# hangxu0304/DeepReduce

Hardware: NVIDIA H100
Metric: ResNet-50 images/sec (whole job, device-timed, max over ranks) (higher is better)
Workload: dtype bf16

## Files before the change

### deepreduce_b200/models/fused_bn.py

```python
from __future__ import annotations

import os

import torch
import torch.nn as nn
import torch.nn.functional as F


def enabled() -> bool:
    return os.environ.get("DR_FUSED_BN", "1") != "0"


def _eligible_x(x: torch.Tensor) -> bool:
    return (x.is_cuda and x.dtype == torch.bfloat16 and x.dim() == 4 and x.stride(1) == 1
            and x.is_contiguous(memory_format=torch.channels_last) and x.size(1) % 8 == 0 and x.size(1) <= 8192
            and x.numel() < 2 ** 31 - 1 and x.numel() // x.size(1) > 1)


def _eligible_bn(bn: nn.BatchNorm2d) -> bool:
    return (bn.training and bn.track_running_stats and bn.running_mean is not None and bn.momentum is not None
            and bn.affine)


def eligible(x: torch.Tensor, bn: nn.BatchNorm2d) -> bool:
    return enabled() and _eligible_x(x) and _eligible_bn(bn)


def _stats(x, bn):
    from .. import ops
    bn.num_batches_tracked.add_(1)
    return ops.cuda_module().bn_stats(x, bn.running_mean, bn.running_var, float(bn.momentum), float(bn.eps))


def _grad(go):
    return go.contiguous(memory_format=torch.channels_last)


def _fork(ctx, o, fork):
    if not fork:
        return o
    ctx.set_materialize_grads(False)
    return o, o.detach()


def _grads(grads):
    gs = [_grad(g) for g in grads if g is not None]
    return (gs + [None, None])[:2]


class _BNReLU(torch.autograd.Function):
    @staticmethod
    def forward(ctx, x, weight, bias, mean, invstd):
        from .. import ops
        y, mask = ops.cuda_module().bn_apply(0, x, [mean, invstd, weight, bias])
        ctx.save_for_backward(x, weight, mean, invstd, mask)
        return y

    @staticmethod
    def backward(ctx, gy):
        from .. import ops
        x, weight, mean, invstd, mask = ctx.saved_tensors
        dx, dw, db = ops.cuda_module().bn_backward(0, _grad(gy), mask, x, [mean, invstd, weight])
        return dx, dw, db, None, None


class _BNAddReLU(torch.autograd.Function):

    @staticmethod
    def forward(ctx, x, weight, bias, mean, invstd, z, wz, bz, mz, iz, fork):
        from .. import ops
        mod = ops.cuda_module()
        if wz is None:
            o, mask = mod.bn_apply(1, x, [mean, invstd, weight, bias], z)
            ctx.save_for_backward(x, weight, mean, invstd, mask)
        else:
            o, mask = mod.bn_apply(2, x, [mean, invstd, weight, bias], z, [mz, iz, wz, bz])
            ctx.save_for_backward(x, weight, mean, invstd, mask, z, wz, mz, iz)
        ctx.has_bn_z = wz is not None
        return _fork(ctx, o, fork)

    @staticmethod
    def backward(ctx, *grads):
        from .. import ops
        mod = ops.cuda_module()
        go, go2 = _grads(grads)
        if go is None:
            return (None,) * 11
        saved = ctx.saved_tensors
        x, weight, mean, invstd, mask = saved[:5]
        if not ctx.has_bn_z:
            dx, dw, db, g = mod.bn_backward(1, go, mask, x, [mean, invstd, weight], go2=go2)
            return dx, dw, db, None, None, g, None, None, None, None, None
        z, wz, mz, iz = saved[5:]
        dx, dw, db, dz, dwz, dbz = mod.bn_backward(2, go, mask, x, [mean, invstd, weight], z, [mz, iz, wz], go2=go2)
        return dx, dw, db, None, None, dz, dwz, dbz, None, None, None


class _BNReLUMaxPool(torch.autograd.Function):

    @staticmethod
    def forward(ctx, x, weight, bias, mean, invstd, fork):
        from .. import ops
        out, codes = ops.cuda_module().bn_apply_pool(x, [mean, invstd, weight, bias])
        ctx.save_for_backward(x, weight, mean, invstd, codes)
        return _fork(ctx, out, fork)

    @staticmethod
    def backward(ctx, *grads):
        from .. import ops
        go, go2 = _grads(grads)
        if go is None:
            return (None,) * 6
        x, weight, mean, invstd, codes = ctx.saved_tensors
        dx, dw, db = ops.cuda_module().bn_backward(3, go, codes, x, [mean, invstd, weight], go2=go2)
        return dx, dw, db, None, None, None


def _stem_pool(pool: nn.Module) -> bool:
    if type(pool) is not nn.MaxPool2d:
        return False
    pair = lambda v: tuple(v) if isinstance(v, (tuple, list)) else (v, v)
    return (pair(pool.kernel_size) == (3, 3) and pair(pool.stride) == (2, 2) and pair(pool.padding) == (1, 1)
            and pair(pool.dilation) == (1, 1) and not pool.ceil_mode and not pool.return_indices)


def _pair(o, fork):
    return (o, o) if fork else o


def bn_relu_maxpool(x: torch.Tensor, bn: nn.BatchNorm2d, pool: nn.MaxPool2d, fork: bool = False):
    if not (eligible(x, bn) and _stem_pool(pool)):
        return _pair(pool(F.relu(bn(x), inplace=True)), fork)
    mean, invstd = _stats(x, bn)
    return _BNReLUMaxPool.apply(x, bn.weight, bn.bias, mean, invstd, fork)


def bn_relu(x: torch.Tensor, bn: nn.BatchNorm2d) -> torch.Tensor:
    if not eligible(x, bn):
        return F.relu(bn(x), inplace=True)
    mean, invstd = _stats(x, bn)
    return _BNReLU.apply(x, bn.weight, bn.bias, mean, invstd)


def bn_add_relu(x: torch.Tensor, bn: nn.BatchNorm2d, idt: torch.Tensor, fork: bool = False):
    if not (eligible(x, bn) and idt.dtype == x.dtype and idt.shape == x.shape and idt.stride() == x.stride()):
        return _pair(F.relu(bn(x) + idt, inplace=True), fork)
    mean, invstd = _stats(x, bn)
    return _BNAddReLU.apply(x, bn.weight, bn.bias, mean, invstd, idt, None, None, None, None, fork)


def bn_bn_add_relu(x: torch.Tensor, bn: nn.BatchNorm2d, xd: torch.Tensor, bnd: nn.BatchNorm2d, fork: bool = False):
    if not (eligible(x, bn) and eligible(xd, bnd) and xd.shape == x.shape and xd.stride() == x.stride()):
        return _pair(F.relu(bn(x) + bnd(xd), inplace=True), fork)
    md, id_ = _stats(xd, bnd)
    mean, invstd = _stats(x, bn)
    return _BNAddReLU.apply(x, bn.weight, bn.bias, mean, invstd, xd, bnd.weight, bnd.bias, md, id_, fork)
```

### deepreduce_b200/models/resnet.py

```python
from __future__ import annotations

import torch.nn as nn
import torch.nn.functional as F

from .fused_bn import bn_add_relu, bn_bn_add_relu, bn_relu, bn_relu_maxpool


class _BasicCifar(nn.Module):
    def __init__(self, inp, out, stride):
        super().__init__()
        self.conv1 = nn.Conv2d(inp, out, 3, stride, 1, bias=False)
        self.bn1 = nn.BatchNorm2d(out)
        self.conv2 = nn.Conv2d(out, out, 3, 1, 1, bias=False)
        self.bn2 = nn.BatchNorm2d(out)
        self.pad = None
        if stride != 1 or inp != out:
            self.pad = (out - inp, stride)

    def forward(self, x):
        y = F.relu(self.bn1(self.conv1(x)))
        y = self.bn2(self.conv2(y))
        if self.pad is not None:
            extra, s = self.pad
            x = F.pad(x[:, :, ::s, ::s], (0, 0, 0, 0, extra // 2, extra - extra // 2))
        return F.relu(x + y)


class ResNetCifar(nn.Module):
    def __init__(self, n: int = 3, num_classes: int = 10):
        super().__init__()
        self.conv1 = nn.Conv2d(3, 16, 3, 1, 1, bias=False)
        self.bn1 = nn.BatchNorm2d(16)
        layers, inp = [], 16
        for out, stride in ((16, 1), (32, 2), (64, 2)):
            for i in range(n):
                layers.append(_BasicCifar(inp, out, stride if i == 0 else 1))
                inp = out
        self.layers = nn.Sequential(*layers)
        self.fc = nn.Linear(64, num_classes)

    def forward(self, x):
        x = F.relu(self.bn1(self.conv1(x)))
        x = self.layers(x)
        x = F.adaptive_avg_pool2d(x, 1).flatten(1)
        return self.fc(x)


def resnet20(num_classes: int = 10) -> ResNetCifar:
    return ResNetCifar(3, num_classes)


class _Bottleneck(nn.Module):
    expansion = 4

    def __init__(self, inp, width, stride, downsample):
        super().__init__()
        out = width * self.expansion
        self.conv1 = nn.Conv2d(inp, width, 1, bias=False)
        self.bn1 = nn.BatchNorm2d(width)
        self.conv2 = nn.Conv2d(width, width, 3, stride, 1, bias=False)
        self.bn2 = nn.BatchNorm2d(width)
        self.conv3 = nn.Conv2d(width, out, 1, bias=False)
        self.bn3 = nn.BatchNorm2d(out)
        self.downsample = None
        if downsample:
            self.downsample = nn.Sequential(nn.Conv2d(inp, out, 1, stride, bias=False), nn.BatchNorm2d(out))

    def forward(self, x, skip=None, fork=False):
        skip = x if skip is None else skip
        xd = None if self.downsample is None else self.downsample[0](skip)
        y = bn_relu(self.conv1(x), self.bn1)
        y = bn_relu(self.conv2(y), self.bn2)
        y = self.conv3(y)
        if xd is None:
            return bn_add_relu(y, self.bn3, skip, fork=fork)
        o = bn_bn_add_relu(y, self.bn3, xd, self.downsample[1])
        return (o, None) if fork else o


class ResNet(nn.Module):
    def __init__(self, blocks=(3, 4, 6, 3), num_classes: int = 1000):
        super().__init__()
        self.conv1 = nn.Conv2d(3, 64, 7, 2, 3, bias=False)
        self.bn1 = nn.BatchNorm2d(64)
        self.maxpool = nn.MaxPool2d(3, 2, 1)
        stages, inp = [], 64
        for i, (n, width) in enumerate(zip(blocks, (64, 128, 256, 512))):
            for j in range(n):
                stride = 2 if (j == 0 and i > 0) else 1
                stages.append(_Bottleneck(inp, width, stride, downsample=(j == 0)))
                inp = width * 4
        self.layers = nn.Sequential(*stages)
        self.fc = nn.Linear(inp, num_classes)
        for m in self.modules():
            if isinstance(m, nn.Conv2d):
                nn.init.kaiming_normal_(m.weight, mode="fan_out", nonlinearity="relu")

    def forward(self, x):
        x, skip = bn_relu_maxpool(self.conv1(x), self.bn1, self.maxpool), None
        for blk in self.layers:
            x, skip = blk(x, skip, fork=True)
        x = F.adaptive_avg_pool2d(x, 1).flatten(1)
        return self.fc(x)


def resnet50(num_classes: int = 1000) -> ResNet:
    return ResNet((3, 4, 6, 3), num_classes)
```

### deepreduce_b200/ops/build.py

```python
from __future__ import annotations

import hashlib
import os
import shutil
import subprocess
import sysconfig
from concurrent.futures import ThreadPoolExecutor

HERE = os.path.dirname(os.path.abspath(__file__))
CSRC = os.path.join(HERE, "csrc")
OBJ = os.path.join(HERE, "build")

CUDA_SOURCES = ["engine.cu", "ops.cu", "p2p.cu", "bn.cu", "p2.cu", "repack.cu"]
NVCC_FLAGS = ["-gencode", "arch=compute_90a,code=sm_90a", "-lineinfo", "-O3", "-std=c++17",
              "--expt-relaxed-constexpr", "--expt-extended-lambda", "-Xcompiler", "-fPIC", "-Xptxas", "-v"]


def _run(cmd, log=None):
    r = subprocess.run(cmd, stdout=subprocess.PIPE, stderr=subprocess.STDOUT, text=True)
    if log is not None:
        with open(log, "w") as f:
            f.write(" ".join(cmd) + "\n" + r.stdout)
    if r.returncode != 0:
        raise RuntimeError("command failed:\n" + " ".join(cmd) + "\n" + r.stdout[-6000:])
    return r.stdout


def _stale(target, sources, extra=""):
    stamp = target + ".stamp"
    h = hashlib.sha256(extra.encode())
    for s in sources:
        with open(s, "rb") as f:
            h.update(f.read())
    digest = h.hexdigest()
    if os.path.exists(target) and os.path.exists(stamp) and open(stamp).read() == digest:
        return False, digest, stamp
    return True, digest, stamp


def _headers():
    return [os.path.join(CSRC, f) for f in os.listdir(CSRC) if f.endswith((".h", ".cuh"))]


def build_cpu(verbose=True):
    import pybind11
    src = os.path.join(CSRC, "cpu", "native_cpu.cpp")
    out = os.path.join(HERE, "_dr_cpu.so")
    stale, digest, stamp = _stale(out, [src])
    if not stale:
        return out
    os.makedirs(OBJ, exist_ok=True)
    cmd = ["g++", "-O3", "-std=c++17", "-shared", "-fPIC", "-fvisibility=hidden",
           "-I", pybind11.get_include(), "-I", sysconfig.get_paths()["include"], src, "-o", out]
    _run(cmd, os.path.join(OBJ, "cpu.log"))
    open(stamp, "w").write(digest)
    if verbose:
        print(f"[build] {out}")
    return out


def build_cuda(verbose=True):
    import torch
    from torch.utils import cpp_extension as ce
    nvcc = shutil.which("nvcc") or "/usr/local/cuda/bin/nvcc"
    out = os.path.join(HERE, "_dr_cuda.so")
    srcs = [os.path.join(CSRC, s) for s in CUDA_SOURCES] + [os.path.join(CSRC, "binding.cpp")]
    stale, digest, stamp = _stale(out, srcs + _headers(), extra=torch.__version__ + " ".join(NVCC_FLAGS))
    if not stale:
        return out
    os.makedirs(OBJ, exist_ok=True)
    abi = int(torch._C._GLIBCXX_USE_CXX11_ABI)

    def cu(src):
        o = os.path.join(OBJ, os.path.basename(src) + ".o")
        _run([nvcc] + NVCC_FLAGS + ["-I", CSRC, "-c", src, "-o", o], os.path.join(OBJ, os.path.basename(src) + ".log"))
        return o

    def cpp(src):
        o = os.path.join(OBJ, "binding.o")
        inc = []
        for p in ce.include_paths("cuda"):
            inc += ["-isystem", p]
        cmd = ["g++", "-O2", "-std=c++17", "-fPIC", "-c", src, "-o", o, "-I", CSRC,
               "-I", sysconfig.get_paths()["include"], f"-D_GLIBCXX_USE_CXX11_ABI={abi}",
               "-DTORCH_EXTENSION_NAME=_dr_cuda", "-DTORCH_API_INCLUDE_EXTENSION_H", "-w"] + inc
        _run(cmd, os.path.join(OBJ, "binding.log"))
        return o

    with ThreadPoolExecutor(max_workers=4) as ex:
        futs = [ex.submit(cu, s) for s in srcs[:-1]] + [ex.submit(cpp, srcs[-1])]
        objs = [f.result() for f in futs]
    libdirs = ce.library_paths("cuda")
    link = ["g++", "-shared", "-o", out] + objs
    for d in libdirs:
        link += ["-L", d, f"-Wl,-rpath,{d}"]
    link += ["-lc10", "-lc10_cuda", "-ltorch_cpu", "-ltorch_cuda", "-ltorch", "-ltorch_python", "-lcudart"]
    _run(link, os.path.join(OBJ, "link.log"))
    open(stamp, "w").write(digest)
    if verbose:
        print(f"[build] {out}")
    return out


def build_all(verbose=True):
    return build_cpu(verbose), build_cuda(verbose)


if __name__ == "__main__":
    build_all()
    for f in sorted(os.listdir(OBJ)):
        if f.endswith(".cu.log"):
            txt = open(os.path.join(OBJ, f)).read()
            for line in txt.splitlines():
                if "registers" in line or "Compiling entry" in line or "spill" in line:
                    print(line)
```

### deepreduce_b200/ops/csrc/binding.cpp

```cpp
#include <ATen/cuda/CUDAContext.h>
#include <c10/cuda/CUDAGuard.h>
#include <c10/cuda/CUDAStream.h>
#include <torch/extension.h>

#include <algorithm>
#include <condition_variable>
#include <deque>
#include <mutex>
#include <thread>

#include "ops.h"

namespace py = pybind11;
using dr::EngineParams;

#define CHECK_CUDA_T(x) TORCH_CHECK((x).is_cuda() && (x).is_contiguous(), #x " must be a contiguous CUDA tensor")

static cudaStream_t cur_stream() { return at::cuda::getCurrentCUDAStream().stream(); }

static void check_last(const char* what) {
  cudaError_t e = cudaGetLastError();
  TORCH_CHECK(e == cudaSuccess, what, ": ", cudaGetErrorString(e));
}

static torch::Tensor bloom_insert(torch::Tensor idx, int64_t k, int64_t m_bits, int64_t seed) {
  CHECK_CUDA_T(idx);
  TORCH_CHECK(idx.scalar_type() == torch::kInt64, "idx must be int64");
  c10::cuda::CUDAGuard g(idx.device());
  const int64_t n_words = (m_bits + 31) / 32;
  auto words = torch::zeros({n_words}, idx.options().dtype(torch::kInt32));
  dr::launch_bloom_insert(idx.data_ptr<int64_t>(), idx.numel(), (uint32_t*)words.data_ptr<int32_t>(), (uint32_t)k,
                          (uint32_t)m_bits, (uint32_t)seed, cur_stream());
  check_last("bloom_insert");
  return words;
}

static torch::Tensor bloom_select(torch::Tensor words, int64_t d, int64_t limit, int64_t k, int64_t m_bits, int64_t seed) {
  CHECK_CUDA_T(words);
  c10::cuda::CUDAGuard g(words.device());
  const int64_t n_tiles = (d + dr::kTile - 1) / dr::kTile;
  auto opts32 = words.options().dtype(torch::kInt32);
  auto counts = torch::empty({n_tiles}, opts32);
  auto excl = torch::empty({n_tiles + 1}, opts32);
  const uint32_t* f = (const uint32_t*)words.data_ptr<int32_t>();
  dr::launch_bloom_count(f, (uint32_t)d, (uint32_t)k, (uint32_t)m_bits, (uint32_t)seed,
                         (uint32_t*)counts.data_ptr<int32_t>(), (uint32_t*)excl.data_ptr<int32_t>(), cur_stream());
  const int64_t total = excl[n_tiles].item<int32_t>();
  const int64_t n_out = (limit < 0) ? total : std::min<int64_t>(limit, total);
  auto out = torch::empty({n_out}, words.options().dtype(torch::kInt64));
  if (n_out > 0)
    dr::launch_bloom_emit(f, (uint32_t)d, (uint32_t)k, (uint32_t)m_bits, (uint32_t)seed,
                          (const uint32_t*)excl.data_ptr<int32_t>(), out.data_ptr<int64_t>(), (uint32_t)n_out, cur_stream());
  check_last("bloom_select");
  return out;
}

static std::vector<torch::Tensor> qsgd_encode(torch::Tensor vals, int64_t q, int64_t bucket, int64_t seed) {
  CHECK_CUDA_T(vals);
  c10::cuda::CUDAGuard g(vals.device());
  auto v = vals.to(torch::kFloat32).contiguous();
  const int64_t K = v.numel();
  const bool i16 = q >= 128;
  auto lvl = torch::empty({K}, v.options().dtype(i16 ? torch::kInt16 : torch::kInt8));
  auto norms = torch::empty({(K + bucket - 1) / bucket}, v.options());
  dr::launch_qsgd_encode(v.data_ptr<float>(), K, (int)bucket, (int)q, (uint32_t)seed, lvl.data_ptr(), i16,
                         norms.data_ptr<float>(), cur_stream());
  check_last("qsgd_encode");
  return {lvl, norms};
}

static torch::Tensor qsgd_decode(torch::Tensor lvl, torch::Tensor norms, int64_t q, int64_t bucket) {
  CHECK_CUDA_T(lvl); CHECK_CUDA_T(norms);
  c10::cuda::CUDAGuard g(lvl.device());
  const bool i16 = lvl.scalar_type() == torch::kInt16;
  auto out = torch::empty({lvl.numel()}, norms.options());
  dr::launch_qsgd_decode(lvl.data_ptr(), i16, norms.data_ptr<float>(), lvl.numel(), (int)bucket, (int)q,
                         out.data_ptr<float>(), cur_stream());
  check_last("qsgd_decode");
  return out;
}

static torch::Tensor pack_bits(torch::Tensor vals, int64_t bits) {
  CHECK_CUDA_T(vals);
  TORCH_CHECK(1 <= bits && bits <= 63, "pack_bits: bits must be in [1, 63], got ", bits);
  c10::cuda::CUDAGuard g(vals.device());
  auto v = vals.to(torch::kInt64).contiguous();
  const int64_t n = v.numel();
  const int64_t n_bytes = (n * bits + 7) / 8, n_words = (n * bits + 31) / 32;
  auto out = torch::empty({n_words}, v.options().dtype(torch::kInt32));
  dr::launch_pack_bits(v.data_ptr<int64_t>(), n, (int)bits, (uint32_t*)out.data_ptr<int32_t>(), n_words, cur_stream());
  check_last("pack_bits");
  return out.view(torch::kUInt8).slice(0, 0, n_bytes);
}

static torch::Tensor unpack_bits(torch::Tensor buf, int64_t n, int64_t bits) {
  CHECK_CUDA_T(buf);
  TORCH_CHECK(1 <= bits && bits <= 63, "unpack_bits: bits must be in [1, 63], got ", bits);
  c10::cuda::CUDAGuard g(buf.device());
  const int64_t n_words = (n * bits + 31) / 32;
  auto padded = torch::zeros({n_words * 4}, buf.options().dtype(torch::kUInt8));
  padded.slice(0, 0, buf.numel()).copy_(buf);
  auto out = torch::empty({n}, buf.options().dtype(torch::kInt64));
  dr::launch_unpack_bits((const uint32_t*)padded.data_ptr<uint8_t>(), n_words, n, (int)bits, out.data_ptr<int64_t>(),
                         cur_stream());
  check_last("unpack_bits");
  return out;
}

static torch::Tensor polyfit_fit(torch::Tensor y, torch::Tensor seg_off, torch::Tensor seg_len, int64_t degree, int64_t max_seg) {
  CHECK_CUDA_T(y); CHECK_CUDA_T(seg_off); CHECK_CUDA_T(seg_len);
  c10::cuda::CUDAGuard g(y.device());
  auto coeffs = torch::zeros({max_seg * (degree + 1)}, y.options());
  dr::launch_polyfit_fit(y.data_ptr<float>(), seg_off.data_ptr<int>(), seg_len.data_ptr<int>(), (int)seg_len.numel(),
                         (int)degree, coeffs.data_ptr<float>(), cur_stream());
  check_last("polyfit_fit");
  return coeffs;
}

static torch::Tensor polyfit_eval(torch::Tensor coeffs, torch::Tensor seg_off, torch::Tensor seg_len, int64_t degree, int64_t total) {
  CHECK_CUDA_T(coeffs);
  c10::cuda::CUDAGuard g(coeffs.device());
  auto out = torch::empty({total}, coeffs.options());
  dr::launch_polyfit_eval(coeffs.data_ptr<float>(), seg_off.data_ptr<int>(), seg_len.data_ptr<int>(),
                          (int)seg_len.numel(), (int)degree, total, out.data_ptr<float>(), cur_stream());
  check_last("polyfit_eval");
  return out;
}

static torch::Tensor conflict_sets_pick(torch::Tensor set_off, torch::Tensor members, torch::Tensor last, int64_t n_pos, int64_t K,
                                        int64_t pseed) {
  CHECK_CUDA_T(set_off); CHECK_CUDA_T(members); CHECK_CUDA_T(last);
  c10::cuda::CUDAGuard g(set_off.device());
  auto out = torch::zeros({(n_pos + 31) / 32}, set_off.options().dtype(torch::kInt32));
  cudaError_t e = dr::launch_conflict_sets_pick((const uint32_t*)set_off.data_ptr<int32_t>(), (const uint32_t*)members.data_ptr<int32_t>(),
                                                (uint32_t*)last.data_ptr<int32_t>(), (uint32_t)(set_off.numel() - 1), (uint32_t)n_pos,
                                                (uint32_t)K, (uint32_t)pseed, (uint32_t*)out.data_ptr<int32_t>(), cur_stream());
  TORCH_CHECK(e == cudaSuccess, "conflict_sets_pick: ", cudaGetErrorString(e));
  return out;
}

static torch::Tensor dexp_fit(torch::Tensor y) {
  CHECK_CUDA_T(y);
  c10::cuda::CUDAGuard g(y.device());
  auto v = y.to(torch::kFloat32).contiguous();
  auto out = torch::zeros({4}, v.options().dtype(torch::kFloat64));
  dr::launch_dexp_fit(v.data_ptr<float>(), v.numel(), out.data_ptr<double>(), cur_stream());
  check_last("dexp_fit");
  return out;
}

static torch::Tensor delta_bp128_encode(torch::Tensor idx) {
  CHECK_CUDA_T(idx);
  c10::cuda::CUDAGuard g(idx.device());
  const int64_t n = idx.numel();
  const int64_t nb = (n + 127) / 128;
  auto widths = torch::zeros({nb}, idx.options().dtype(torch::kInt32));
  dr::launch_bp128_widths(idx.data_ptr<int64_t>(), n, (uint32_t*)widths.data_ptr<int32_t>(), cur_stream());
  auto sizes = widths.to(torch::kInt64) * 4 + 1;
  auto incl = sizes.cumsum(0);
  auto off = (incl - sizes).contiguous();
  const int64_t total = nb ? incl[nb - 1].item<int64_t>() : 0;
  auto out = torch::zeros({total}, idx.options().dtype(torch::kInt32));
  dr::launch_bp128_pack(idx.data_ptr<int64_t>(), n, (const uint32_t*)widths.data_ptr<int32_t>(), off.data_ptr<int64_t>(),
                        (uint32_t*)out.data_ptr<int32_t>(), cur_stream());
  check_last("delta_bp128_encode");
  return out;
}

static torch::Tensor delta_bp128_decode(torch::Tensor payload, int64_t n) {
  CHECK_CUDA_T(payload);
  c10::cuda::CUDAGuard g(payload.device());
  const int64_t nb = (n + 127) / 128;
  auto off = torch::empty({nb + 1}, payload.options().dtype(torch::kInt64));
  auto deltas = torch::empty({n}, payload.options().dtype(torch::kInt64));
  dr::launch_bp128_unpack((const uint32_t*)payload.data_ptr<int32_t>(), n, off.data_ptr<int64_t>(),
                          deltas.data_ptr<int64_t>(), cur_stream());
  check_last("delta_bp128_decode");
  return deltas.cumsum(0);
}

static torch::Tensor rle_runs(torch::Tensor idx, int64_t d) {
  CHECK_CUDA_T(idx);
  c10::cuda::CUDAGuard g(idx.device());
  const int64_t n = idx.numel();
  auto o64 = idx.options().dtype(torch::kInt64);
  if (n == 0) return torch::full({1}, d, o64);
  const int64_t nb = (n + 1023) / 1024;
  auto counts = torch::empty({nb}, idx.options().dtype(torch::kInt32));
  auto excl = torch::empty({nb + 1}, idx.options().dtype(torch::kInt32));
  dr::launch_rle_count(idx.data_ptr<int64_t>(), n, (uint32_t*)counts.data_ptr<int32_t>(), (uint32_t*)excl.data_ptr<int32_t>(),
                       cur_stream());
  const int64_t n_runs = excl[nb].item<int32_t>();
  auto start_pos = torch::empty({n_runs}, o64), end_pos = torch::empty({n_runs}, o64);
  auto runs = torch::zeros({2 * n_runs + 1}, o64);
  dr::launch_rle_runs(idx.data_ptr<int64_t>(), n, (const uint32_t*)excl.data_ptr<int32_t>(), start_pos.data_ptr<int64_t>(),
                      end_pos.data_ptr<int64_t>(), n_runs, d, runs.data_ptr<int64_t>(), cur_stream());
  check_last("rle_runs");
  const int64_t last = idx[n - 1].item<int64_t>();
  return (d - 1 - last > 0) ? runs : runs.slice(0, 0, 2 * n_runs);
}

static torch::Tensor rle_indices(torch::Tensor runs) {
  CHECK_CUDA_T(runs);
  c10::cuda::CUDAGuard g(runs.device());
  const int64_t n_pairs = runs.numel() / 2;
  auto o64 = runs.options().dtype(torch::kInt64);
  if (n_pairs == 0) return torch::empty({0}, o64);
  auto pairs = runs.slice(0, 0, 2 * n_pairs).to(torch::kInt64).view({n_pairs, 2});
  auto z = pairs.select(1, 0), o = pairs.select(1, 1);
  auto csum = (z + o).cumsum(0);
  auto run_start = (csum - o).contiguous();
  auto ones_incl = o.cumsum(0);
  auto ones_excl = (ones_incl - o).contiguous();
  const int64_t total = ones_incl[n_pairs - 1].item<int64_t>();
  auto out = torch::empty({total}, o64);
  dr::launch_rle_expand(ones_excl.data_ptr<int64_t>(), run_start.data_ptr<int64_t>(), n_pairs, total, out.data_ptr<int64_t>(),
                        cur_stream());
  check_last("rle_indices");
  return out;
}

static torch::Tensor u8_to_nhwc_norm(torch::Tensor in, std::vector<double> mean, std::vector<double> stdv) {
  CHECK_CUDA_T(in);
  TORCH_CHECK(in.scalar_type() == torch::kUInt8 && in.size(-1) == 3, "expect uint8 [...,3] NHWC");
  c10::cuda::CUDAGuard g(in.device());
  in = in.contiguous();
  if (reinterpret_cast<uintptr_t>(in.data_ptr()) % 4 != 0) in = in.clone(at::MemoryFormat::Contiguous);
  auto out = torch::empty(in.sizes(), in.options().dtype(torch::kBFloat16));
  float m[3] = {(float)mean[0], (float)mean[1], (float)mean[2]};
  float s[3] = {(float)(1.0 / stdv[0]), (float)(1.0 / stdv[1]), (float)(1.0 / stdv[2])};
  dr::launch_u8_to_nhwc_norm(in.data_ptr<uint8_t>(), out.data_ptr(), in.numel() / 3, m, s, cur_stream());
  check_last("u8_to_nhwc_norm");
  return out;
}

struct Repack {
  torch::Tensor table;
  int64_t n_seg = 0, n_vec = 0, ddp_numel = 0, eng_numel = 0;
  int elem_bytes = 0;
  c10::ScalarType dtype;

  Repack(torch::Tensor segs, int64_t ddp_numel_, int64_t eng_numel_, torch::Tensor like)
      : ddp_numel(ddp_numel_), eng_numel(eng_numel_), dtype(like.scalar_type()) {
    TORCH_CHECK(dtype == torch::kFloat32 || dtype == torch::kBFloat16, "Repack: fp32 or bf16 buckets, got ", dtype);
    TORCH_CHECK(like.is_cuda(), "Repack: the buckets must be CUDA tensors");
    const torch::Device device = like.device();
    TORCH_CHECK(!segs.is_cuda() && segs.scalar_type() == torch::kInt64 && segs.dim() == 2 && segs.size(1) == 3,
                "Repack: segments must be a host int64 tensor [n, 3] of {ddp_off, eng_off, numel}");
    elem_bytes = dtype == torch::kFloat32 ? 4 : 2;
    const int64_t V = 16 / elem_bytes;
    segs = segs.contiguous();
    n_seg = segs.size(0);
    TORCH_CHECK(n_seg < (1 << 30), "Repack: too many segments");
    auto host = torch::empty({n_seg + 1, 4}, torch::kInt64);
    const int64_t* s = segs.data_ptr<int64_t>();
    int64_t* h = host.data_ptr<int64_t>();
    std::vector<std::pair<int64_t, int64_t>> ddp_ranges, eng_ranges;
    for (int64_t i = 0; i < n_seg; ++i) {
      const int64_t d = s[3 * i], e = s[3 * i + 1], n = s[3 * i + 2];
      TORCH_CHECK(n > 0, "Repack: segment ", i, " is empty");
      TORCH_CHECK(d >= 0 && d + n <= ddp_numel, "Repack: segment ", i, " [", d, ", ", d + n,
                  ") lies outside the DDP buffer of ", ddp_numel, " elements");
      TORCH_CHECK(e >= 0 && e % V == 0, "Repack: segment ", i, " starts at engine element ", e,
                  ", not on a 16-byte vector");
      TORCH_CHECK((e + n + V - 1) / V * V <= eng_numel, "Repack: segment ", i, " [", e, ", ", e + n,
                  ") lies outside the engine buffer of ", eng_numel, " elements");
      h[4 * i] = d; h[4 * i + 1] = e; h[4 * i + 2] = n; h[4 * i + 3] = n_vec;
      n_vec += (n + V - 1) / V;
      ddp_ranges.emplace_back(d, d + n);
      eng_ranges.emplace_back(e, e + n);
    }
    h[4 * n_seg] = 0; h[4 * n_seg + 1] = 0; h[4 * n_seg + 2] = 0; h[4 * n_seg + 3] = n_vec;
    for (auto* r : {&ddp_ranges, &eng_ranges}) {
      std::sort(r->begin(), r->end());
      for (size_t i = 1; i < r->size(); ++i)
        TORCH_CHECK((*r)[i].first >= (*r)[i - 1].second, "Repack: segments overlap at element ", (*r)[i].first);
    }
    table = host.to(device);
  }

  void check_buffers(const torch::Tensor& ddp, const torch::Tensor& eng) const {
    for (const torch::Tensor* t : {&ddp, &eng}) {
      TORCH_CHECK(t->is_cuda() && t->is_contiguous() && t->dim() == 1, "Repack: buffers are contiguous 1-D CUDA tensors");
      TORCH_CHECK(t->scalar_type() == dtype, "Repack: the table was built for ", dtype, " buffers, got ", t->scalar_type());
      TORCH_CHECK(t->device() == table.device(), "Repack: buffer on ", t->device(), ", table on ", table.device());
    }
    TORCH_CHECK(ddp.numel() >= ddp_numel, "Repack: the DDP buffer has ", ddp.numel(), " elements, the table needs ", ddp_numel);
    TORCH_CHECK(eng.numel() >= eng_numel, "Repack: the engine buffer has ", eng.numel(), " elements, the table needs ", eng_numel);
    TORCH_CHECK(reinterpret_cast<uintptr_t>(eng.data_ptr()) % 16 == 0, "Repack: the engine buffer must be 16-byte aligned");
  }

  void pack(torch::Tensor ddp, torch::Tensor eng) const {
    check_buffers(ddp, eng);
    c10::cuda::CUDAGuard g(eng.device());
    cudaError_t e = dr::launch_bucket_repack(true, elem_bytes, ddp.data_ptr(), eng.data_ptr(), table.data_ptr<int64_t>(),
                                             (int)n_seg, n_vec, cur_stream());
    TORCH_CHECK(e == cudaSuccess, "bucket_pack: ", cudaGetErrorString(e));
  }

  void unpack(torch::Tensor eng, torch::Tensor ddp) const {
    check_buffers(ddp, eng);
    c10::cuda::CUDAGuard g(eng.device());
    cudaError_t e = dr::launch_bucket_repack(false, elem_bytes, eng.data_ptr(), ddp.data_ptr(), table.data_ptr<int64_t>(),
                                             (int)n_seg, n_vec, cur_stream());
    TORCH_CHECK(e == cudaSuccess, "bucket_unpack: ", cudaGetErrorString(e));
  }
};

namespace at::native {
struct Var;
template <typename scalar_t, typename VarTransform>
void batch_norm_stats_channels_last_cuda_template(const at::Tensor& out_mean, const at::Tensor& out_invstd,
                                                   const at::Tensor& input, double epsilon);
}

static void check_bn_input(const torch::Tensor& x) {
  TORCH_CHECK(x.is_cuda() && x.scalar_type() == torch::kBFloat16 && x.dim() == 4 && x.stride(1) == 1 &&
                  x.is_contiguous(at::MemoryFormat::ChannelsLast),
              "bn: x must be a channels_last bf16 CUDA tensor");
  TORCH_CHECK(x.size(1) % 8 == 0 && x.size(1) <= 8192, "bn: channels must be a multiple of 8, at most 8192");
  TORCH_CHECK(x.numel() < std::numeric_limits<int32_t>::max(), "bn: tensor too large for 32-bit indexing");
}

static void check_chan(const torch::Tensor& t, int64_t C, const char* what) {
  TORCH_CHECK(t.is_cuda() && t.scalar_type() == torch::kFloat32 && t.is_contiguous() && t.numel() == C, "bn: ", what,
              " must be a contiguous float32 CUDA tensor of C elements");
}

static std::vector<torch::Tensor> bn_stats(torch::Tensor x, torch::Tensor running_mean, torch::Tensor running_var,
                                           double momentum, double eps, bool torch_kernel) {
  check_bn_input(x);
  const int64_t C = x.size(1);
  check_chan(running_mean, C, "running_mean");
  check_chan(running_var, C, "running_var");
  const int64_t N = x.numel() / C;
  TORCH_CHECK(N > 1, "bn: expected more than 1 value per channel when training");
  c10::cuda::CUDAGuard g(x.device());
  auto opts = x.options().dtype(torch::kFloat32);
  auto mean = torch::empty({C}, opts), invstd = torch::empty({C}, opts);
  const float bessel = static_cast<float>(static_cast<double>(N) / static_cast<double>(N - 1));
  int block_y = 0, grid_y = 0;
  dr::bn_row_tree(N, (int)C, &block_y, &grid_y);
  cudaError_t e;
  if (!torch_kernel && (int64_t)block_y * grid_y <= N) {
    auto staging = grid_y > 1 ? torch::empty({(2 * C + 1) * grid_y}, opts) : torch::Tensor();
    const dr::BnStats s{x.data_ptr(), mean.data_ptr<float>(), invstd.data_ptr<float>(), running_mean.data_ptr<float>(),
                        running_var.data_ptr<float>(), grid_y > 1 ? staging.data_ptr<float>() : nullptr,
                        (float)momentum, bessel, (float)eps};
    e = dr::launch_bn_stats(s, N, (int)C, cur_stream());
  } else {
    at::native::batch_norm_stats_channels_last_cuda_template<c10::BFloat16, at::native::Var>(mean, invstd, x, eps);
    e = dr::launch_bn_update_stats(mean.data_ptr<float>(), invstd.data_ptr<float>(), running_mean.data_ptr<float>(),
                                   running_var.data_ptr<float>(), (int)C, (float)momentum, bessel, (float)eps,
                                   cur_stream());
  }
  TORCH_CHECK(e == cudaSuccess, "bn_stats: ", cudaGetErrorString(e));
  return {mean, invstd};
}

static dr::BnParams bn_params(const std::vector<torch::Tensor>& p, int64_t C) {
  TORCH_CHECK(p.size() == 4, "bn: expected (mean, invstd, weight, bias)");
  const char* names[4] = {"mean", "invstd", "weight", "bias"};
  for (int i = 0; i < 4; ++i) check_chan(p[i], C, names[i]);
  return {p[0].data_ptr<float>(), p[1].data_ptr<float>(), p[2].data_ptr<float>(), p[3].data_ptr<float>()};
}

static void check_like_x(const torch::Tensor& t, const torch::Tensor& x, const char* what) {
  TORCH_CHECK(t.sizes() == x.sizes() && t.strides() == x.strides() && t.scalar_type() == torch::kBFloat16 &&
                  t.device() == x.device(),
              "bn: ", what, " must match x in shape, layout, dtype and device");
}

static std::vector<torch::Tensor> bn_apply(int64_t mode, torch::Tensor x, std::vector<torch::Tensor> p,
                                           c10::optional<torch::Tensor> z, std::vector<torch::Tensor> pz) {
  check_bn_input(x);
  const int64_t C = x.size(1);
  const dr::BnParams px = bn_params(p, C);
  dr::BnParams pzz{};
  const void* zp = nullptr;
  if (mode != 0) {
    TORCH_CHECK(z.has_value(), "bn: mode ", mode, " needs z");
    check_like_x(*z, x, "z");
    zp = z->data_ptr();
    if (mode == 2) pzz = bn_params(pz, C);
  }
  c10::cuda::CUDAGuard g(x.device());
  const int64_t rows = x.numel() / C;
  auto out = torch::empty_like(x);
  auto mask = torch::empty({rows, C / 8}, x.options().dtype(torch::kUInt8));
  cudaError_t e = dr::launch_bn_apply((int)mode, x.data_ptr(), px, zp, pzz, out.data_ptr(), mask.data_ptr(), rows,
                                      (int)C, cur_stream());
  TORCH_CHECK(e == cudaSuccess, "bn_apply: ", cudaGetErrorString(e));
  return {out, mask};
}

static std::vector<torch::Tensor> bn_apply_pool(torch::Tensor x, std::vector<torch::Tensor> p, int64_t kernel_size,
                                                int64_t stride, int64_t padding, int64_t dilation, bool ceil_mode) {
  TORCH_CHECK(kernel_size == 3 && stride == 2 && padding == 1 && dilation == 1 && !ceil_mode,
              "bn_apply_pool: only kernel 3, stride 2, padding 1, dilation 1, floor mode");
  check_bn_input(x);
  const int64_t N = x.size(0), C = x.size(1), H = x.size(2), W = x.size(3);
  const dr::BnParams px = bn_params(p, C);
  c10::cuda::CUDAGuard g(x.device());
  const dr::PoolGeom pg{(int)H, (int)W, (int)((H - 1) / 2 + 1), (int)((W - 1) / 2 + 1)};
  auto out = torch::empty({N, C, pg.Ho, pg.Wo}, x.options().memory_format(at::MemoryFormat::ChannelsLast));
  auto codes = torch::empty({N * pg.Ho * pg.Wo, C}, x.options().dtype(torch::kUInt8));
  cudaError_t e = dr::launch_bn_apply_pool(x.data_ptr(), px, out.data_ptr(), codes.data_ptr(), (int)N, pg, (int)C,
                                           cur_stream());
  TORCH_CHECK(e == cudaSuccess, "bn_apply_pool: ", cudaGetErrorString(e));
  return {out, codes};
}

static dr::BnParams bn_bwd_params(const std::vector<torch::Tensor>& p, int64_t C) {
  TORCH_CHECK(p.size() == 3, "bn_backward: expected (mean, invstd, weight)");
  const char* names[3] = {"mean", "invstd", "weight"};
  for (int i = 0; i < 3; ++i) check_chan(p[i], C, names[i]);
  return {p[0].data_ptr<float>(), p[1].data_ptr<float>(), p[2].data_ptr<float>(), nullptr};
}

static std::vector<torch::Tensor> bn_backward(int64_t mode, torch::Tensor go, torch::Tensor mask, torch::Tensor x,
                                              std::vector<torch::Tensor> p, c10::optional<torch::Tensor> z,
                                              std::vector<torch::Tensor> pz, c10::optional<torch::Tensor> go2) {
  TORCH_CHECK(mode >= 0 && mode <= 3, "bn_backward: mode must be 0, 1, 2 or 3");
  TORCH_CHECK(!go2.has_value() || mode != 0, "bn_backward: mode 0 takes no go2");
  check_bn_input(x);
  const int64_t C = x.size(1), rows = x.numel() / C;
  dr::PoolGeom pg{(int)x.size(2), (int)x.size(3), (int)((x.size(2) - 1) / 2 + 1), (int)((x.size(3) - 1) / 2 + 1)};
  const std::vector<int64_t> go_shape =
      mode == 3 ? std::vector<int64_t>{x.size(0), C, pg.Ho, pg.Wo} : x.sizes().vec();
  for (const torch::Tensor* t : {&go, go2.has_value() ? &*go2 : &go})
    TORCH_CHECK(t->sizes() == go_shape && t->scalar_type() == torch::kBFloat16 && t->device() == x.device() &&
                    t->is_contiguous(at::MemoryFormat::ChannelsLast),
                "bn_backward: go and go2 must be channels_last bf16 tensors on x's device, of x's shape (mode 3: the "
                "pooled shape)");
  const int64_t mask_numel = mode == 3 ? go.numel() : rows * (C / 8);
  TORCH_CHECK(mask.is_cuda() && mask.scalar_type() == torch::kUInt8 && mask.is_contiguous() &&
                  mask.numel() == mask_numel && mask.device() == x.device(),
              "bn_backward: mask must be bn_apply's mask (mode 3: bn_apply_pool's codes) for x");
  c10::cuda::CUDAGuard guard(x.device());
  int block_y = 0, grid_y = 0;
  dr::bn_row_tree(rows, (int)C, &block_y, &grid_y);
  TORCH_CHECK((int64_t)block_y * grid_y <= rows, "bn_backward: reduction tree wider than the rows");
  const int n_sums = mode == 2 ? 3 : 2;
  auto f32 = x.options().dtype(torch::kFloat32);
  auto sums = torch::empty({n_sums, C}, f32);
  auto staging = grid_y > 1 ? torch::empty({n_sums, grid_y, C}, f32) : torch::Tensor();
  auto dx = torch::empty_like(x), dw = torch::empty({C}, f32), db = torch::empty({C}, f32);
  dr::BnBwd b{};
  b.go = go.data_ptr(); b.go2 = go2.has_value() ? go2->data_ptr() : nullptr; b.mask = mask.data_ptr<uint8_t>(); b.x = x.data_ptr();
  b.px = bn_bwd_params(p, C);
  b.dx = dx.data_ptr(); b.sums = sums.data_ptr<float>(); b.staging = grid_y > 1 ? staging.data_ptr<float>() : nullptr;
  b.dw = dw.data_ptr<float>(); b.db = db.data_ptr<float>();
  b.pool = pg;
  std::vector<torch::Tensor> res{dx, dw, db};
  torch::Tensor g;
  if (mode == 1 || mode == 3) {
    g = torch::empty_like(x);
    b.g = g.data_ptr();
    if (mode == 1) res.push_back(g);
  } else if (mode == 2) {
    TORCH_CHECK(z.has_value(), "bn_backward: mode 2 needs z");
    check_like_x(*z, x, "z");
    b.z = z->data_ptr();
    b.pz = bn_bwd_params(pz, C);
    auto dz = torch::empty_like(x), dwz = torch::empty({C}, f32), dbz = torch::empty({C}, f32);
    b.dz = dz.data_ptr(); b.dwz = dwz.data_ptr<float>(); b.dbz = dbz.data_ptr<float>();
    res.insert(res.end(), {dz, dwz, dbz});
  }
  cudaError_t e = dr::launch_bn_backward((int)mode, b, rows, (int)C, cur_stream());
  TORCH_CHECK(e == cudaSuccess, "bn_backward: ", cudaGetErrorString(e));
  return res;
}

struct Engine {
  EngineParams P{};
  int grid = 0;
  int grid_cap = 0;
  int blocks_per_sm = 2;
  int dyn_smem = 64 * 1024;
  int device = 0;
  const dr::P2Entry* p2_entries = nullptr;
  uint32_t n_p2 = 0, p2_max_pos_cap = 0;
  uint32_t* p2_scratch = nullptr;

  Engine(int64_t tensors, int64_t tiles, int64_t n_tensors, int64_t n_tiles, int64_t slot_words,
         int64_t payload_words, int64_t grad, int64_t resid, int64_t hist, int64_t hist_total, int64_t sel,
         int64_t tile_count, int64_t barrier, int64_t status, std::vector<int64_t> arenas, int rank, int world) {
    TORCH_CHECK(world <= dr::kMaxWorld && (int)arenas.size() == world, "bad world/arenas");
    P.tensors = reinterpret_cast<const dr::TensorDesc*>(tensors);
    P.tiles = reinterpret_cast<const dr::TileInfo*>(tiles);
    P.n_tensors = (uint32_t)n_tensors; P.n_tiles = (uint32_t)n_tiles;
    P.slot_words = (uint32_t)slot_words; P.payload_words = (uint32_t)payload_words;
    P.grad = reinterpret_cast<float*>(grad); P.resid = reinterpret_cast<float*>(resid);
    P.hist = reinterpret_cast<uint32_t*>(hist); P.hist_total = reinterpret_cast<uint32_t*>(hist_total);
    P.sel = reinterpret_cast<dr::SelState*>(sel);
    P.tile_count = reinterpret_cast<uint32_t*>(tile_count);
    P.barrier = reinterpret_cast<uint32_t*>(barrier); P.status = reinterpret_cast<uint32_t*>(status);
    for (int i = 0; i < world; ++i) P.arena[i] = reinterpret_cast<uint32_t*>(arenas[i]);
    P.rank = rank; P.world = world;
    P.beta = 1.f; P.gamma = 1.f; P.scale = 1.f / world; P.seed = dr::kDefaultSeed; P.policy = 0; P.use_history = 1;
    P.spin_limit = 20u * 1000u * 1000u;
    P.filter_smem_words = (uint32_t)(dyn_smem / 4);
    P.use_tma = 1; P.hist_shift = 23;
    P.shard = 0; P.s2_words = 0; P.s2_cap = 0; P.has_rle = 0; P.has_shared = 0; P.has_bf16_values = 0; P.mc_arena = nullptr;
    P.peer_timeout_ms = 120000u; P.fault = 0; P.debug_times = nullptr; P.cost_prefix = nullptr; P.deterministic = 0; P.cuts = nullptr; P.cuts_grid = 0;
    cudaGetDevice(&device);
  }

  void configure(double beta, double gamma, double scale, int64_t seed, int policy, int use_history, int64_t spin_limit,
                 int bps, int64_t filter_smem_bytes, int use_tma, int hist_shift) {
    P.beta = (float)beta; P.gamma = (float)gamma; P.scale = (float)scale; P.seed = (uint32_t)seed;
    P.policy = policy; P.use_history = use_history; P.spin_limit = (uint32_t)spin_limit;
    blocks_per_sm = bps; grid = 0;
    dyn_smem = (int)filter_smem_bytes; P.filter_smem_words = (uint32_t)(dyn_smem / 4);
    P.use_tma = use_tma; P.hist_shift = (uint32_t)hist_shift;
  }

  void set_poly(int64_t tensors, int64_t n_poly, int64_t tasks, int64_t n_tasks, int64_t bins, int64_t bucket_val,
                int64_t bucket_pos, int64_t expand_buf, int64_t poly_total) {
    P.poly_tensors = reinterpret_cast<const uint32_t*>(tensors); P.n_poly = (uint32_t)n_poly;
    P.poly_tasks = reinterpret_cast<const uint32_t*>(tasks); P.n_poly_tasks = (uint32_t)n_tasks;
    P.poly_bins = reinterpret_cast<uint32_t*>(bins); P.bucket_val = reinterpret_cast<float*>(bucket_val);
    P.bucket_pos = reinterpret_cast<uint32_t*>(bucket_pos); P.expand_buf = reinterpret_cast<float*>(expand_buf);
    P.poly_total = (uint32_t)poly_total;
  }

  void set_p2(int64_t entries, int64_t n, int64_t scratch, int64_t max_pos_cap) {
    TORCH_CHECK(n == 0 || (entries && scratch), "set_p2: null table or scratch");
    TORCH_CHECK((size_t)((max_pos_cap + 31) / 32) * 4 <= dr::kP2MaxSmemBytes, "set_p2: pos_cap ", max_pos_cap,
                " exceeds what the draw holds in shared memory");
    if (n) {
      c10::cuda::CUDAGuard guard((c10::DeviceIndex)device);
      const cudaError_t e = dr::p2_prepare();
      TORCH_CHECK(e == cudaSuccess, "set_p2: ", cudaGetErrorString(e));
    }
    p2_entries = reinterpret_cast<const dr::P2Entry*>(entries); n_p2 = (uint32_t)n;
    p2_scratch = reinterpret_cast<uint32_t*>(scratch); p2_max_pos_cap = (uint32_t)max_pos_cap;
  }

  void set_has_rle(int v) { P.has_rle = v; }
  void set_has_shared(int v) { P.has_shared = v; }
  void set_has_bf16_values(int v) { P.has_bf16_values = v; }
  void set_scratch(int64_t pos_mask, int64_t dec_mask, int64_t cand, int64_t cand_cnt) {
    P.pos_mask = reinterpret_cast<uint32_t*>(pos_mask); P.dec_mask = reinterpret_cast<uint32_t*>(dec_mask);
    P.cand = reinterpret_cast<uint2*>(cand); P.cand_cnt = reinterpret_cast<uint32_t*>(cand_cnt);
  }
  void set_peer_timeout_ms(int64_t ms) { P.peer_timeout_ms = (uint32_t)ms; }
  void set_fault(int f) { P.fault = f; }
  void set_deterministic(int d) { P.deterministic = d; }
  void set_cost_prefix(int64_t p) { P.cost_prefix = reinterpret_cast<const uint32_t*>(p); }
  void set_debug_times(int64_t p) { P.debug_times = reinterpret_cast<unsigned long long*>(p); }
  void set_cuts(int64_t p, int64_t grid) { P.cuts = reinterpret_cast<const uint32_t*>(p); P.cuts_grid = (uint32_t)grid; }
  void set_grid_cap(int cap) { grid_cap = cap; }
  void set_multicast(int64_t p) { P.mc_arena = reinterpret_cast<uint32_t*>(p); }

  void set_shard(int shard, int64_t s2_words, int64_t s2_cap) {
    P.shard = shard; P.s2_words = (uint32_t)s2_words; P.s2_cap = (uint32_t)s2_cap;
  }

  void set_bf16(int64_t grad_bf16, int64_t acc32, int64_t acc_tiles) {
    TORCH_CHECK(grad_bf16 != 0, "set_bf16: null gradient");
    TORCH_CHECK(acc_tiles == 0 || acc32 != 0, "set_bf16: null accumulator");
    P.grad_bf16 = reinterpret_cast<uint16_t*>(grad_bf16); P.acc32 = reinterpret_cast<float*>(acc32);
    P.acc_tiles = (uint32_t)acc_tiles; P.bf16 = 1;
  }

  void set_buffers(int64_t grad, int64_t resid) {
    P.grad = reinterpret_cast<float*>(grad); P.resid = reinterpret_cast<float*>(resid);
  }

  void set_momentum(int64_t mom, double momentum) {
    P.mom = reinterpret_cast<float*>(mom); P.momentum = (float)momentum;
  }

  void set_weight_decay(int64_t table, double weight_decay) {
    TORCH_CHECK(weight_decay == 0.0 || table != 0, "set_weight_decay: weight decay needs the parameter table");
    P.wparams = reinterpret_cast<const unsigned long long*>(table); P.weight_decay = (float)weight_decay;
  }

  int get_grid() {
    if (grid == 0) grid = dr::engine_max_grid(blocks_per_sm, dyn_smem);
    return grid;
  }

  void run_on(uint32_t epoch, int phase_begin, int phase_end, cudaStream_t st) {
    if (n_p2 == 0) { launch_range(epoch, phase_begin, phase_end, st); return; }
    const uint32_t parity = epoch & 1u;
    uint32_t* slots = P.arena[P.rank] + dr::slot_offset(P, parity, 0);
    dr::P2Args A{P.tensors, P.tiles, p2_entries, n_p2, p2_scratch, P.pos_mask, P.tile_count,
                 P.arena[P.rank] + dr::slot_offset(P, parity, P.rank), epoch, P.seed};
    int b = phase_begin;
    auto upto = [&](int e) { if (b < e) launch_range(epoch, b, e, st); b = e; };
    auto check = [](cudaError_t e, const char* what) { TORCH_CHECK(e == cudaSuccess, what, ": ", cudaGetErrorString(e)); };
    if (phase_begin <= dr::kPhEmit && dr::kPhEmit < phase_end) {
      upto(dr::kPhEmit);
      check(dr::p2_pick_launch(A, p2_max_pos_cap, st), "P2 pick launch failed");
      upto(dr::kPhEmit + 1);
      check(dr::p2_header_launch(A, st), "P2 header launch failed");
    }
    if (P.world > 1 && phase_begin <= dr::kPhCompact && dr::kPhCompact < phase_end) {
      upto(dr::kPhCompact);
      uint32_t s_begin, s_end;
      dr::decode_span(P, P.rank, s_begin, s_end);
      dr::P2Thin T{P.tensors, P.tiles, slots, P.slot_words, P.dec_mask, P.rank, P.world, s_begin, s_end - s_begin};
      check(dr::p2_thin_launch(T, st), "P2 thin launch failed");
    }
    upto(phase_end);
  }

  void launch_range(uint32_t epoch, int phase_begin, int phase_end, cudaStream_t st) {
    EngineParams Q = P;
    Q.epoch = epoch; Q.phase_begin = phase_begin; Q.phase_end = phase_end;
    TORCH_CHECK(P.pos_mask && P.cand, "Engine: set_scratch() was not called");
    if (P.bf16 && P.acc_tiles) {
      uint32_t s_begin, s_end;
      dr::decode_span(P, P.rank, s_begin, s_end);
      const uint32_t span = s_end - s_begin;
      TORCH_CHECK(P.acc_tiles >= span, "Engine: the bf16 accumulator covers ", P.acc_tiles, " tiles, the decode span ", span);
    }
    int g = get_grid();
    if (grid_cap > 0 && grid_cap < g) g = grid_cap;
    cudaError_t e = dr::engine_launch(Q, g, blocks_per_sm, dyn_smem, st);
    TORCH_CHECK(e == cudaSuccess, "engine launch failed: ", cudaGetErrorString(e));
  }

  void run(int64_t epoch, int phase_begin, int phase_end) { run_on((uint32_t)epoch, phase_begin, phase_end, cur_stream()); }
};

struct Scheduler {
  struct Item { Engine* eng; uint32_t epoch; cudaEvent_t ready; cudaEvent_t done; };
  std::thread worker;
  std::mutex mu;
  std::condition_variable cv, cv_done;
  std::deque<Item> q;
  bool stop = false;
  int64_t submitted = 0, completed = 0;
  cudaStream_t side = nullptr;
  int device = 0;
  std::vector<cudaEvent_t> ready_ev, done_ev;
  std::string error;

  explicit Scheduler(int n_buckets) {
    cudaGetDevice(&device);
    int lo = 0, hi = 0;
    cudaDeviceGetStreamPriorityRange(&lo, &hi);
    cudaStreamCreateWithPriority(&side, cudaStreamNonBlocking, hi);
    ready_ev.resize(n_buckets); done_ev.resize(n_buckets);
    for (int i = 0; i < n_buckets; ++i) {
      cudaEventCreateWithFlags(&ready_ev[i], cudaEventDisableTiming);
      cudaEventCreateWithFlags(&done_ev[i], cudaEventDisableTiming);
    }
    worker = std::thread([this] { loop(); });
  }

  ~Scheduler() { shutdown(); }

  void shutdown() {
    {
      std::lock_guard<std::mutex> l(mu);
      if (stop) return;
      stop = true;
    }
    cv.notify_all();
    if (worker.joinable()) worker.join();
    for (auto e : ready_ev) cudaEventDestroy(e);
    for (auto e : done_ev) cudaEventDestroy(e);
    if (side) cudaStreamDestroy(side);
    side = nullptr;
  }

  void loop() {
    cudaSetDevice(device);
    while (true) {
      Item it;
      {
        std::unique_lock<std::mutex> l(mu);
        cv.wait(l, [this] { return stop || !q.empty(); });
        if (q.empty()) return;
        it = q.front(); q.pop_front();
      }
      cudaStreamWaitEvent(side, it.ready, 0);
      try {
        it.eng->run_on(it.epoch, dr::kPhAccum, dr::kPhEnd, side);
      } catch (const std::exception& ex) {
        std::lock_guard<std::mutex> l(mu);
        error = ex.what();
      }
      cudaEventRecord(it.done, side);
      {
        std::lock_guard<std::mutex> l(mu);
        ++completed;
      }
      cv_done.notify_all();
    }
  }

  void submit(int bucket, Engine* eng, int64_t epoch) {
    cudaEventRecord(ready_ev[bucket], cur_stream());
    {
      std::lock_guard<std::mutex> l(mu);
      q.push_back(Item{eng, (uint32_t)epoch, ready_ev[bucket], done_ev[bucket]});
      ++submitted;
    }
    cv.notify_one();
  }

  void wait_all() {
    py::gil_scoped_release rel;
    {
      std::unique_lock<std::mutex> l(mu);
      cv_done.wait(l, [this] { return completed == submitted; });
      TORCH_CHECK(error.empty(), "background engine launch failed: ", error);
    }
    for (auto e : done_ev) cudaStreamWaitEvent(cur_stream(), e, 0);
  }
};

static int64_t arena_alloc(int64_t bytes) {
  void* p = dr::arena_alloc((size_t)bytes);
  TORCH_CHECK(p != nullptr, "arena cudaMalloc failed");
  return (int64_t)p;
}
static py::bytes arena_export(int64_t p) {
  dr::ArenaHandle h = dr::arena_export((void*)p);
  return py::bytes((const char*)h.bytes, sizeof(h.bytes));
}
static int64_t arena_import(const std::string& b) {
  TORCH_CHECK(b.size() == sizeof(dr::ArenaHandle), "bad handle");
  dr::ArenaHandle h;
  memcpy(h.bytes, b.data(), sizeof(h.bytes));
  void* p = dr::arena_import(h);
  TORCH_CHECK(p != nullptr, "cudaIpcOpenMemHandle failed (peer access / IPC unavailable)");
  return (int64_t)p;
}
static torch::Tensor arena_as_tensor(int64_t p, int64_t n_words, int64_t device) {
  auto opts = torch::TensorOptions().dtype(torch::kInt32).device(torch::kCUDA, (int)device);
  return torch::from_blob((void*)p, {n_words}, opts);
}

PYBIND11_MODULE(TORCH_EXTENSION_NAME, m) {
  m.def("launch_count", [] { return (int64_t)dr::launch_count(); });
  m.def("bloom_insert", &bloom_insert);
  m.def("bloom_select", &bloom_select);
  m.def("qsgd_encode", &qsgd_encode);
  m.def("qsgd_decode", &qsgd_decode);
  m.def("pack_bits", &pack_bits);
  m.def("unpack_bits", &unpack_bits);
  m.def("polyfit_fit", &polyfit_fit);
  m.def("polyfit_eval", &polyfit_eval);
  m.def("dexp_fit", &dexp_fit);
  m.def("conflict_sets_pick", &conflict_sets_pick);
  m.def("delta_bp128_encode", &delta_bp128_encode);
  m.def("delta_bp128_decode", &delta_bp128_decode);
  m.def("u8_to_nhwc_norm", &u8_to_nhwc_norm);
  m.def("bn_stats", &bn_stats, py::arg("x"), py::arg("running_mean"), py::arg("running_var"), py::arg("momentum"),
        py::arg("eps"), py::arg("torch_kernel") = false);
  m.def("bn_apply", &bn_apply, py::arg("mode"), py::arg("x"), py::arg("p"), py::arg("z") = py::none(),
        py::arg("pz") = std::vector<torch::Tensor>{});
  m.def("bn_apply_pool", &bn_apply_pool, py::arg("x"), py::arg("p"), py::arg("kernel_size") = 3, py::arg("stride") = 2,
        py::arg("padding") = 1, py::arg("dilation") = 1, py::arg("ceil_mode") = false);
  m.def("bn_backward", &bn_backward, py::arg("mode"), py::arg("go"), py::arg("mask"), py::arg("x"), py::arg("p"),
        py::arg("z") = py::none(), py::arg("pz") = std::vector<torch::Tensor>{}, py::arg("go2") = py::none());
  m.def("rle_runs", &rle_runs);
  m.def("rle_indices", &rle_indices);
  m.def("arena_alloc", &arena_alloc);
  m.def("arena_free", [](int64_t p) { dr::arena_free((void*)p); });
  m.def("arena_export", &arena_export);
  m.def("arena_import", &arena_import);
  m.def("arena_close", [](int64_t p) { dr::arena_close((void*)p); });
  m.def("arena_as_tensor", &arena_as_tensor);
  m.def("enable_peer_access", [](std::vector<int> devices) { return dr::arena_enable_peer_access(devices.data(), (int)devices.size()); });
  py::class_<Repack>(m, "Repack")
      .def(py::init<torch::Tensor, int64_t, int64_t, torch::Tensor>(), py::arg("segments"), py::arg("ddp_numel"),
           py::arg("eng_numel"), py::arg("like"))
      .def("pack", &Repack::pack, py::arg("ddp"), py::arg("eng"))
      .def("unpack", &Repack::unpack, py::arg("eng"), py::arg("ddp"))
      .def_readonly("table", &Repack::table)
      .def_readonly("n_seg", &Repack::n_seg)
      .def_readonly("n_vec", &Repack::n_vec);
  m.attr("TILE") = dr::kTile;
  m.attr("ARENA_HDR_WORDS") = dr::kArenaHdrWords;
  m.attr("SLOT_HEADER_WORDS") = dr::kSlotHeaderWords;
  m.attr("HIST_BINS") = dr::kHistBins;
  m.attr("NUM_HIST") = dr::kNumHist;
  m.attr("PH_END") = (int)dr::kPhEnd;

  py::class_<Engine>(m, "Engine")
      .def(py::init<int64_t, int64_t, int64_t, int64_t, int64_t, int64_t, int64_t, int64_t, int64_t, int64_t, int64_t,
                    int64_t, int64_t, int64_t, std::vector<int64_t>, int, int>())
      .def("configure", &Engine::configure)
      .def("set_buffers", &Engine::set_buffers)
      .def("set_momentum", &Engine::set_momentum)
      .def("set_weight_decay", &Engine::set_weight_decay)
      .def("set_bf16", &Engine::set_bf16)
      .def("set_poly", &Engine::set_poly)
      .def("set_shard", &Engine::set_shard)
      .def("set_has_rle", &Engine::set_has_rle)
      .def("set_p2", &Engine::set_p2)
      .def("set_has_shared", &Engine::set_has_shared)
      .def("set_has_bf16_values", &Engine::set_has_bf16_values)
      .def("set_scratch", &Engine::set_scratch)
      .def("set_peer_timeout_ms", &Engine::set_peer_timeout_ms)
      .def("set_fault", &Engine::set_fault)
      .def("set_deterministic", &Engine::set_deterministic)
      .def("set_cost_prefix", &Engine::set_cost_prefix)
      .def("set_debug_times", &Engine::set_debug_times)
      .def("set_cuts", &Engine::set_cuts)
      .def("set_grid_cap", &Engine::set_grid_cap)
      .def("set_multicast", &Engine::set_multicast)
      .def("grid", &Engine::get_grid)
      .def("run", &Engine::run);

  py::class_<Scheduler>(m, "Scheduler")
      .def(py::init<int>())
      .def("submit", &Scheduler::submit)
      .def("wait_all", &Scheduler::wait_all)
      .def("shutdown", &Scheduler::shutdown);
}
```

### deepreduce_b200/ops/csrc/bn.cu

```cuda
#include <cuda_bf16.h>

#include <algorithm>

#include "common.cuh"
#include "ops.h"

namespace dr {

namespace {

constexpr int kVec = 8;
constexpr int kApplyThreads = 256;
constexpr int kReduceThreads = 128;

struct ChanParams {
  float m[kVec], inv[kVec], w[kVec], b[kVec];
};

__device__ __forceinline__ void load8(const float* __restrict__ p, float* d) {
  const float4 a = __ldg(reinterpret_cast<const float4*>(p));
  const float4 b = __ldg(reinterpret_cast<const float4*>(p) + 1);
  d[0] = a.x; d[1] = a.y; d[2] = a.z; d[3] = a.w;
  d[4] = b.x; d[5] = b.y; d[6] = b.z; d[7] = b.w;
}

__device__ __forceinline__ void load_params(const BnParams& p, int c, ChanParams& o) {
  load8(p.mean + c, o.m);
  load8(p.invstd + c, o.inv);
  load8(p.weight + c, o.w);
  load8(p.bias + c, o.b);
}

__device__ __forceinline__ float bn_elem(float x, float m, float inv, float w, float b) {
  return __fmaf_rn(__fmul_rn(w, __fsub_rn(x, m)), inv, b);
}

__device__ __forceinline__ __nv_bfloat16 relu_bf16(__nv_bfloat16 v) {
  return __bfloat162float(v) <= 0.f ? __float2bfloat16_rn(0.f) : v;
}

__device__ __forceinline__ uint4 add_bf16x8(const uint4& a, const uint4& b) {
  uint4 s;
  const __nv_bfloat16* ha = reinterpret_cast<const __nv_bfloat16*>(&a);
  const __nv_bfloat16* hb = reinterpret_cast<const __nv_bfloat16*>(&b);
  __nv_bfloat16* hs = reinterpret_cast<__nv_bfloat16*>(&s);
#pragma unroll
  for (int i = 0; i < kVec; ++i) hs[i] = __float2bfloat16_rn(__fadd_rn(__bfloat162float(ha[i]), __bfloat162float(hb[i])));
  return s;
}

template <int kMode>
__global__ void __launch_bounds__(kApplyThreads) bn_apply_kernel(const __nv_bfloat16* __restrict__ x, BnParams px,
                                                                 const __nv_bfloat16* __restrict__ z, BnParams pz,
                                                                 __nv_bfloat16* __restrict__ out,
                                                                 uint8_t* __restrict__ mask, int64_t rows, int C) {
  const int groups = C / kVec;
  const int rows_per_cta = blockDim.x / groups;
  const int rsub = threadIdx.x / groups;
  if (rsub >= rows_per_cta) return;
  const int c = (threadIdx.x % groups) * kVec;
  ChanParams a;
  load_params(px, c, a);
  ChanParams d;
  if (kMode == 2) load_params(pz, c, d);
  const int64_t step = (int64_t)gridDim.x * rows_per_cta;
#pragma unroll 2
  for (int64_t r = (int64_t)blockIdx.x * rows_per_cta + rsub; r < rows; r += step) {
    const int64_t off = r * C + c;
    const uint4 vx = *reinterpret_cast<const uint4*>(x + off);
    uint4 vz = make_uint4(0, 0, 0, 0);
    if (kMode != 0) vz = *reinterpret_cast<const uint4*>(z + off);
    const __nv_bfloat16* hx = reinterpret_cast<const __nv_bfloat16*>(&vx);
    const __nv_bfloat16* hz = reinterpret_cast<const __nv_bfloat16*>(&vz);
    uint4 vo;
    __nv_bfloat16* ho = reinterpret_cast<__nv_bfloat16*>(&vo);
    unsigned bits = 0;
#pragma unroll
    for (int i = 0; i < kVec; ++i) {
      __nv_bfloat16 y = __float2bfloat16_rn(bn_elem(__bfloat162float(hx[i]), a.m[i], a.inv[i], a.w[i], a.b[i]));
      if (kMode != 0) {
        const __nv_bfloat16 s = kMode == 1 ? hz[i]
                                           : __float2bfloat16_rn(bn_elem(__bfloat162float(hz[i]), d.m[i], d.inv[i], d.w[i], d.b[i]));
        y = __float2bfloat16_rn(__fadd_rn(__bfloat162float(y), __bfloat162float(s)));
      }
      ho[i] = relu_bf16(y);
      bits |= (__bfloat162float(ho[i]) <= 0.f ? 0u : 1u) << i;
    }
    *reinterpret_cast<uint4*>(out + off) = vo;
    mask[r * groups + c / kVec] = (uint8_t)bits;
  }
}


__global__ void __launch_bounds__(kApplyThreads) bn_apply_pool_kernel(const __nv_bfloat16* __restrict__ x, BnParams px,
                                                                      __nv_bfloat16* __restrict__ out,
                                                                      uint8_t* __restrict__ codes, int64_t orows,
                                                                      PoolGeom pg, int C) {
  const int groups = C / kVec;
  const int rows_per_cta = blockDim.x / groups;
  const int rsub = threadIdx.x / groups;
  if (rsub >= rows_per_cta) return;
  const int c = (threadIdx.x % groups) * kVec;
  ChanParams a;
  load_params(px, c, a);
  const int64_t step = (int64_t)gridDim.x * rows_per_cta;
  for (int64_t r = (int64_t)blockIdx.x * rows_per_cta + rsub; r < orows; r += step) {
    const int ow = (int)(r % pg.Wo);
    const int64_t t = r / pg.Wo;
    const int oh = (int)(t % pg.Ho);
    const int64_t n = t / pg.Ho;
    const int h0 = 2 * oh - 1, w0 = 2 * ow - 1;
    uint4 v[9];
#pragma unroll
    for (int k = 0; k < 9; ++k) {
      const int ih = h0 + k / 3, iw = w0 + k % 3;
      v[k] = ih >= 0 && ih < pg.H && iw >= 0 && iw < pg.W
                 ? *reinterpret_cast<const uint4*>(x + ((n * pg.H + ih) * pg.W + iw) * C + c)
                 : uint4{};
    }
    __nv_bfloat16 best[kVec];
    unsigned slot[kVec];
#pragma unroll
    for (int i = 0; i < kVec; ++i) {
      best[i] = __float2bfloat16_rn(-INFINITY);
      slot[i] = 0;
    }
#pragma unroll
    for (int k = 0; k < 9; ++k) {
      const int ih = h0 + k / 3, iw = w0 + k % 3;
      if (ih < 0 || ih >= pg.H || iw < 0 || iw >= pg.W) continue;
      const __nv_bfloat16* hx = reinterpret_cast<const __nv_bfloat16*>(&v[k]);
#pragma unroll
      for (int i = 0; i < kVec; ++i) {
        const __nv_bfloat16 y = relu_bf16(__float2bfloat16_rn(bn_elem(__bfloat162float(hx[i]), a.m[i], a.inv[i], a.w[i], a.b[i])));
        const float fy = __bfloat162float(y);
        if (fy > __bfloat162float(best[i]) || isnan(fy)) {
          best[i] = y;
          slot[i] = k;
        }
      }
    }
    uint4 vo;
    __nv_bfloat16* ho = reinterpret_cast<__nv_bfloat16*>(&vo);
    uint2 vc;
    uint8_t* hc = reinterpret_cast<uint8_t*>(&vc);
#pragma unroll
    for (int i = 0; i < kVec; ++i) {
      ho[i] = best[i];
      hc[i] = (uint8_t)(slot[i] | (__bfloat162float(best[i]) <= 0.f ? 0u : 0x80u));
    }
    *reinterpret_cast<uint4*>(out + r * C + c) = vo;
    *reinterpret_cast<uint2*>(codes + r * C + c) = vc;
  }
}

struct PoolGather {
  uint4 g[4];
  uint2 code[4];
  int off;
  int nh, nw;
  int sh, sw;
};

__device__ __forceinline__ void pool_gather_codes(PoolGather& q, const uint8_t* __restrict__ codes, const PoolGeom& pg,
                                                  int row, int C, int c, bool valid) {
  const int w = row % pg.W, t = row / pg.W, h = t % pg.H, n = t / pg.H;
  const int ph = h >> 1, pw = w >> 1;
  q.nh = valid ? min((h + 1) / 2 + 1, pg.Ho) - ph : 0;
  q.nw = valid ? min((w + 1) / 2 + 1, pg.Wo) - pw : 0;
  q.sh = h - 2 * ph + 1;
  q.sw = w - 2 * pw + 1;
  q.off = ((n * pg.Ho + ph) * pg.Wo + pw) * C + c;
#pragma unroll
  for (int k = 0; k < 4; ++k) {
    const int a = k >> 1, b = k & 1;
    q.code[k] = a < q.nh && b < q.nw ? *reinterpret_cast<const uint2*>(codes + q.off + (a * pg.Wo + b) * C) : uint2{};
  }
}

template <bool kTwo>
__device__ __forceinline__ void pool_gather_grads(PoolGather& q, const __nv_bfloat16* __restrict__ gp,
                                                  const __nv_bfloat16* __restrict__ gp2, const PoolGeom& pg, int C) {
#pragma unroll
  for (int k = 0; k < 4; ++k) {
    const int a = k >> 1, b = k & 1;
    const bool in = a < q.nh && b < q.nw;
    const int off = q.off + (a * pg.Wo + b) * C;
    q.g[k] = in ? *reinterpret_cast<const uint4*>(gp + off) : uint4{};
    if (kTwo && in) q.g[k] = add_bf16x8(q.g[k], *reinterpret_cast<const uint4*>(gp2 + off));
  }
}

__device__ __forceinline__ void pool_gather_resolve(const PoolGather& q, uint4& g, unsigned& bits) {
  __nv_bfloat16* hg = reinterpret_cast<__nv_bfloat16*>(&g);
  const bool single = q.nh == 1 && q.nw == 1;
  bits = 0;
#pragma unroll
  for (int i = 0; i < kVec; ++i) {
    float s = 0.f;
    __nv_bfloat16 one = __float2bfloat16_rn(0.f);
    unsigned bit = 0;
#pragma unroll
    for (int k = 0; k < 4; ++k) {
      const int a = k >> 1, b = k & 1;
      const unsigned code = (reinterpret_cast<const uint8_t*>(&q.code[k]))[i];
      if (a < q.nh && b < q.nw && (int)(code & 0x7fu) == (q.sh - 2 * a) * 3 + (q.sw - 2 * b)) {
        const __nv_bfloat16 v = (reinterpret_cast<const __nv_bfloat16*>(&q.g[k]))[i];
        s = __fadd_rn(s, __bfloat162float(v));
        one = v;
        bit = code >> 7;
      }
    }
    hg[i] = single ? one : __float2bfloat16_rn(s);
    bits |= bit << i;
  }
}

template <bool kTwo>
__global__ void __launch_bounds__(kApplyThreads) bn_pool_grad_kernel(const __nv_bfloat16* __restrict__ gp,
                                                                     const __nv_bfloat16* __restrict__ gp2,
                                                                     const uint8_t* __restrict__ codes,
                                                                     __nv_bfloat16* __restrict__ g, PoolGeom pg,
                                                                     int64_t rows, int C) {
  const int groups = C / kVec;
  const int rows_per_cta = blockDim.x / groups;
  const int rsub = threadIdx.x / groups;
  if (rsub >= rows_per_cta) return;
  const int c = (threadIdx.x % groups) * kVec;
  const int64_t step = (int64_t)gridDim.x * rows_per_cta;
#pragma unroll 2
  for (int64_t r = (int64_t)blockIdx.x * rows_per_cta + rsub; r < rows; r += step) {
    PoolGather q;
    pool_gather_codes(q, codes, pg, (int)r, C, c, true);
    pool_gather_grads<kTwo>(q, gp, gp2, pg, C);
    uint4 v;
    unsigned bits;
    pool_gather_resolve(q, v, bits);
    __nv_bfloat16* hv = reinterpret_cast<__nv_bfloat16*>(&v);
#pragma unroll
    for (int i = 0; i < kVec; ++i)
      if (!((bits >> i) & 1u)) hv[i] = __float2bfloat16_rn(0.f);
    *reinterpret_cast<uint4*>(g + r * C + c) = v;
  }
}

struct RowTree {
  int block_y, grid_y;
  __host__ __device__ int S() const { return block_y * grid_y; }
  __host__ __device__ int loops(int rows) const { return 1 + (rows - 1) / (S() * kLoads); }
  static constexpr int kLoads = 4;
};

constexpr int kStatsThreads = 256;

__device__ __forceinline__ void welford_update(float x, float inv, float valid, float& mean, float& m2n) {
  const float d0 = __fsub_rn(x, mean);
  mean = __fmaf_rn(d0, inv, mean);
  const float d1 = __fsub_rn(x, mean);
  m2n = __fmaf_rn(__fmul_rn(d0, d1), valid, m2n);
}

template <int kN, bool kFuseNew>
__device__ __forceinline__ void welford_merge(int& n, float* mean, float* m2n, int n_new, const float* mean_new,
                                              const float* m2n_new) {
  const float fn = (float)n, fn_new = (float)n_new;
  const float factor = __frcp_rn((float)max(1, n + n_new));
#pragma unroll
  for (int i = 0; i < kN; ++i) {
    const float d = __fsub_rn(mean[i], mean_new[i]);
    const float s = kFuseNew ? __fmaf_rn(mean_new[i], fn_new, __fmul_rn(mean[i], fn))
                             : __fmaf_rn(mean[i], fn, __fmul_rn(mean_new[i], fn_new));
    mean[i] = __fmul_rn(s, factor);
    const float u = __fmul_rn(__fmul_rn(__fmul_rn(d, d), fn_new), fn);
    m2n[i] = __fadd_rn(m2n[i], __fmaf_rn(u, factor, m2n_new[i]));
  }
  n += n_new;
}

template <int kN>
struct WelfordSlots {
  float* mean; float* m2n; int* count;
  __device__ WelfordSlots(float* sh, int slots)
      : mean(sh), m2n(sh + slots * kN), count(reinterpret_cast<int*>(sh + 2 * slots * kN)) {}
  __device__ void put(int s, int n, const float* m, const float* q) const {
#pragma unroll
    for (int i = 0; i < kN; ++i) { mean[s * kN + i] = m[i]; m2n[s * kN + i] = q[i]; }
    count[s] = n;
  }
  template <bool kFuseNew>
  __device__ void merge_from(int s, int& n, float* m, float* q) const {
    float mn[kN], qn[kN];
#pragma unroll
    for (int i = 0; i < kN; ++i) { mn[i] = mean[s * kN + i]; qn[i] = m2n[s * kN + i]; }
    welford_merge<kN, kFuseNew>(n, m, q, count[s], mn, qn);
  }
  static size_t bytes(int slots) { return (size_t)slots * (2 * kN * sizeof(float) + sizeof(int)); }
};

template <int kN>
__device__ __forceinline__ void welford_tree_over_y(const WelfordSlots<kN>& sl, bool part, int y, int block_y, int base,
                                                    int stride, int& n, float* mean, float* m2n) {
  for (int off = block_y / 2; off > 0; off >>= 1) {
    if (part && y < 2 * off) sl.put(base + y * stride, n, mean, m2n);
    __syncthreads();
    if (part && y < off) sl.template merge_from<false>(base + (y + off) * stride, n, mean, m2n);
    __syncthreads();
  }
}

struct StatsOut {
  float* mean; float* invstd; float* running_mean; float* running_var;
  float* st_mean; float* st_m2n; int* st_count;
  float momentum, bessel, eps;
};

__device__ __forceinline__ void stats_store(const StatsOut& o, int c, int n, float mean, float m2n) {
  const float var = __fdiv_rn(m2n, (float)n);
  const float keep = __fsub_rn(1.f, o.momentum);
  o.mean[c] = mean;
  o.invstd[c] = rsqrtf(__fadd_rn(var, o.eps));
  o.running_mean[c] = __fmaf_rn(mean, o.momentum, __fmul_rn(o.running_mean[c], keep));
  o.running_var[c] = __fmaf_rn(__fmul_rn(var, o.bessel), o.momentum, __fmul_rn(o.running_var[c], keep));
}

__global__ void __launch_bounds__(kStatsThreads) bn_stats_kernel(const __nv_bfloat16* __restrict__ x, StatsOut o,
                                                                 RowTree t, int rows, int C) {
  constexpr int L = RowTree::kLoads;
  constexpr int kAhead = 4;
  extern __shared__ float sh[];
  const int gpc = blockDim.x / (L * t.block_y);
  const int g = threadIdx.x % gpc, j = (threadIdx.x / gpc) % L, y = threadIdx.x / (gpc * L);
  const int group = blockIdx.x * gpc + g;
  const bool live = group * kVec < C;
  const int c = live ? group * kVec : 0;
  const int S = t.S();
  const int n_loops = t.loops(rows);
  const int r0 = blockIdx.y * t.block_y + y + j * S;
  const int rstep = L * S;
  float mean[kVec], m2n[kVec];
#pragma unroll
  for (int i = 0; i < kVec; ++i) mean[i] = m2n[i] = 0.f;
  int n = 0;
  auto load = [&](uint4* b, int i0) {
#pragma unroll
    for (int u = 0; u < kAhead; ++u) {
      const int r = r0 + (i0 + u) * rstep;
      b[u] = live && i0 + u < n_loops && r < rows ? *reinterpret_cast<const uint4*>(x + (size_t)r * C + c) : uint4{};
    }
  };
  uint4 cur[kAhead];
  load(cur, 0);
  for (int i0 = 0; i0 < n_loops; i0 += kAhead) {
    uint4 nxt[kAhead];
    load(nxt, i0 + kAhead);
#pragma unroll
    for (int u = 0; u < kAhead; ++u) {
      const int i = i0 + u;
      if (i >= n_loops) break;
      const bool valid = r0 + i * rstep < rows;
      const float inv = valid ? __frcp_rn((float)(i + 1)) : 0.f;
      const float fv = valid ? 1.f : 0.f;
      n += valid;
      const __nv_bfloat16* hx = reinterpret_cast<const __nv_bfloat16*>(&cur[u]);
#pragma unroll
      for (int k = 0; k < kVec; ++k) welford_update(__bfloat162float(hx[k]), inv, fv, mean[k], m2n[k]);
    }
#pragma unroll
    for (int u = 0; u < kAhead; ++u) cur[u] = nxt[u];
  }
  const WelfordSlots<kVec> sl(sh, blockDim.x);
  sl.put(threadIdx.x, n, mean, m2n);
  __syncthreads();
  if (j == 0) {
#pragma unroll
    for (int a = 1; a < L; ++a) sl.merge_from<true>(threadIdx.x + a * gpc, n, mean, m2n);
  }
  __syncthreads();
  welford_tree_over_y<kVec>(sl, j == 0, y, t.block_y, g, gpc * L, n, mean, m2n);
  if (j != 0 || y != 0 || !live) return;
  if (t.grid_y == 1) {
#pragma unroll
    for (int i = 0; i < kVec; ++i) stats_store(o, c + i, n, mean[i], m2n[i]);
    return;
  }
#pragma unroll
  for (int i = 0; i < kVec; ++i) {
    o.st_mean[(size_t)blockIdx.y * C + c + i] = mean[i];
    o.st_m2n[(size_t)blockIdx.y * C + c + i] = m2n[i];
  }
  if (group == 0) o.st_count[blockIdx.y] = n;
}

__global__ void bn_stats_finalize_kernel(StatsOut o, RowTree t, int C) {
  extern __shared__ float sh[];
  const int cols = blockDim.x / t.block_y;
  const int col = threadIdx.x % cols, y = threadIdx.x / cols;
  const int c = blockIdx.x * cols + col;
  int n = 0;
  float mean = 0.f, m2n = 0.f;
  if (c < C)
    for (int b = y; b < t.grid_y; b += t.block_y) {
      const float mb = o.st_mean[(size_t)b * C + c], qb = o.st_m2n[(size_t)b * C + c];
      welford_merge<1, false>(n, &mean, &m2n, o.st_count[b], &mb, &qb);
    }
  const WelfordSlots<1> sl(sh, blockDim.x);
  welford_tree_over_y<1>(sl, true, y, t.block_y, col, cols, n, &mean, &m2n);
  if (y == 0 && c < C) stats_store(o, c, n, mean, m2n);
}


template <int kN>
__device__ __forceinline__ void tree_over_y(float* v, float* sh, int y, int n, int col, int width) {
  for (int off = n / 2; off > 0; off >>= 1) {
#pragma unroll
    for (int i = 0; i < kN; ++i) sh[y * width + col + i] = v[i];
    __syncthreads();
    if (y < off) {
#pragma unroll
      for (int i = 0; i < kN; ++i) v[i] = __fadd_rn(v[i], sh[(y + off) * width + col + i]);
    }
    __syncthreads();
  }
}

struct BwdOut {
  float* sums;
  float* dw; float* db; float* dwz; float* dbz;
  float* staging;
};

__device__ __forceinline__ void bwd_store(const BwdOut& o, int k, int c, int C, float v, const float* invstd,
                                         const float* invstd_z) {
  o.sums[k * C + c] = v;
  if (k == 0) {
    o.db[c] = v;
    if (o.dbz) o.dbz[c] = v;
  } else if (k == 1) {
    o.dw[c] = __fmul_rn(v, invstd[c]);
  } else {
    o.dwz[c] = __fmul_rn(v, invstd_z[c]);
  }
}

__device__ __forceinline__ float masked(__nv_bfloat16 go, unsigned bit) { return bit ? __bfloat162float(go) : 0.f; }

template <int kMode, bool kTwo>
__global__ void __launch_bounds__(kReduceThreads) bn_bwd_reduce_kernel(const __nv_bfloat16* __restrict__ go,
                                                                       const __nv_bfloat16* __restrict__ go2,
                                                                       const uint8_t* __restrict__ mask,
                                                                       const __nv_bfloat16* __restrict__ x,
                                                                       const float* __restrict__ mean,
                                                                       const float* __restrict__ invstd,
                                                                       const __nv_bfloat16* __restrict__ z,
                                                                       const float* __restrict__ mean_z,
                                                                       const float* __restrict__ invstd_z,
                                                                       __nv_bfloat16* __restrict__ g_out, BwdOut o,
                                                                       RowTree t, int rows, int C) {
  constexpr int kSums = kMode == 2 ? 3 : 2;
  constexpr int L = RowTree::kLoads;
  extern __shared__ float sh[];
  const int gpc = blockDim.x / t.block_y;
  const int tg = threadIdx.x % gpc, y = threadIdx.x / gpc;
  const int group = blockIdx.x * gpc + tg;
  const bool live = group * kVec < C;
  const int c = live ? group * kVec : 0;
  const int S = t.S();
  float m[kVec], mz[kVec];
#pragma unroll
  for (int i = 0; i < kVec; ++i) {
    m[i] = mean[c + i];
    mz[i] = kMode == 2 ? mean_z[c + i] : 0.f;
  }
  float acc[kSums][L][kVec];
#pragma unroll
  for (int k = 0; k < kSums; ++k)
#pragma unroll
    for (int j = 0; j < L; ++j)
#pragma unroll
      for (int i = 0; i < kVec; ++i) acc[k][j][i] = 0.f;
  const int mgroups = C / kVec;
  int r = blockIdx.y * t.block_y + y;
  const int n_loops = t.loops(rows);
  constexpr bool kAhead = !(kTwo && kMode == 2);
  struct Batch {
    uint4 g[L], g2[L], x[L], z[L];
    unsigned m[L];
  };
  auto load = [&](Batch& b, int r0) {
#pragma unroll
    for (int j = 0; j < L; ++j) {
      const int rr = r0 + j * S;
      if (live && rr < rows) {
        const int off = rr * C + c;
        b.g[j] = *reinterpret_cast<const uint4*>(go + off);
        if (kTwo) b.g2[j] = *reinterpret_cast<const uint4*>(go2 + off);
        b.x[j] = *reinterpret_cast<const uint4*>(x + off);
        if (kMode == 2) b.z[j] = *reinterpret_cast<const uint4*>(z + off);
        b.m[j] = kMode == 3 ? 0u : mask[rr * mgroups + group];
      } else {
        b.g[j] = uint4{}; b.g2[j] = uint4{}; b.x[j] = uint4{}; b.z[j] = uint4{}; b.m[j] = 0;
      }
    }
  };
  Batch cur;
  if (kAhead) load(cur, r);
  for (int it = 0; it < n_loops; ++it) {
    if (!kAhead) load(cur, r);
    if (kTwo) {
#pragma unroll
      for (int j = 0; j < L; ++j) cur.g[j] = add_bf16x8(cur.g[j], cur.g2[j]);
    }
    Batch nxt;
    if (kAhead) load(nxt, r + L * S);
    const unsigned* mb = cur.m;
#pragma unroll
    for (int j = 0; j < L; ++j) {
      const __nv_bfloat16* hg = reinterpret_cast<const __nv_bfloat16*>(&cur.g[j]);
      const __nv_bfloat16* hx = reinterpret_cast<const __nv_bfloat16*>(&cur.x[j]);
      const __nv_bfloat16* hz = reinterpret_cast<const __nv_bfloat16*>(&cur.z[j]);
      uint4 vo;
      __nv_bfloat16* ho = reinterpret_cast<__nv_bfloat16*>(&vo);
#pragma unroll
      for (int i = 0; i < kVec; ++i) {
        const unsigned bit = (mb[j] >> i) & 1u;
        const float g = kMode == 3 ? __bfloat162float(hg[i]) : masked(hg[i], bit);
        if (kMode == 1) ho[i] = bit ? hg[i] : __float2bfloat16_rn(0.f);
        acc[0][j][i] = __fadd_rn(acc[0][j][i], g);
        acc[1][j][i] = __fmaf_rn(__fsub_rn(__bfloat162float(hx[i]), m[i]), g, acc[1][j][i]);
        if (kMode == 2) acc[2][j][i] = __fmaf_rn(__fsub_rn(__bfloat162float(hz[i]), mz[i]), g, acc[2][j][i]);
      }
      if (kMode == 1 && live && r + j * S < rows) *reinterpret_cast<uint4*>(g_out + (r + j * S) * C + c) = vo;
    }
    if (kAhead) cur = nxt;
    r += L * S;
  }
#pragma unroll
  for (int k = 0; k < kSums; ++k) {
#pragma unroll
    for (int i = 0; i < kVec; ++i)
#pragma unroll
      for (int j = 1; j < L; ++j) acc[k][0][i] = __fadd_rn(acc[k][0][i], acc[k][j][i]);
    tree_over_y<kVec>(acc[k][0], sh, y, t.block_y, tg * kVec, gpc * kVec);
  }
  if (y != 0 || !live) return;
#pragma unroll
  for (int k = 0; k < kSums; ++k)
#pragma unroll
    for (int i = 0; i < kVec; ++i) {
      if (t.grid_y > 1) o.staging[((size_t)k * t.grid_y + blockIdx.y) * C + c + i] = acc[k][0][i];
      else bwd_store(o, k, c + i, C, acc[k][0][i], invstd, invstd_z);
    }
}

__global__ void bn_bwd_finalize_kernel(BwdOut o, RowTree t, int n_sums, int C, const float* __restrict__ invstd,
                                       const float* __restrict__ invstd_z) {
  extern __shared__ float sh[];
  const int cols = blockDim.x / t.block_y;
  const int col = threadIdx.x % cols, y = threadIdx.x / cols;
  const int c = blockIdx.x * cols + col;
  for (int k = 0; k < n_sums; ++k) {
    float v = 0.f;
    if (c < C)
      for (int b = y; b < t.grid_y; b += t.block_y) v = __fadd_rn(v, o.staging[((size_t)k * t.grid_y + b) * C + c]);
    tree_over_y<1>(&v, sh, y, t.block_y, col, cols);
    if (y == 0 && c < C) bwd_store(o, k, c, C, v, invstd, invstd_z);
  }
}

struct ElemtChan {
  float m[kVec], f1[kVec], f2[kVec], sdy[kVec];
};

__device__ __forceinline__ void elemt_params(const float* mean, const float* invstd, const float* w, const float* sdy,
                                             const float* sxmu, float norm, int c, ElemtChan& p) {
  float inv[kVec], ww[kVec], sx[kVec];
  load8(mean + c, p.m);
  load8(invstd + c, inv);
  load8(w + c, ww);
  load8(sdy + c, p.sdy);
  load8(sxmu + c, sx);
#pragma unroll
  for (int i = 0; i < kVec; ++i) {
    p.f1[i] = __fmul_rn(__fmul_rn(__fmul_rn(inv[i], inv[i]), sx[i]), norm);
    p.f2[i] = __fmul_rn(ww[i], inv[i]);
  }
}

__device__ __forceinline__ __nv_bfloat16 elemt(float g, float x, const ElemtChan& p, int i, float norm) {
  const float a = __fmaf_rn(-p.sdy[i], norm, g);
  return __float2bfloat16_rn(__fmul_rn(__fmaf_rn(-p.f1[i], __fsub_rn(x, p.m[i]), a), p.f2[i]));
}

struct ElemtArgs {
  const float *mean, *invstd, *weight, *sums;
  const float *mean_z, *invstd_z, *weight_z;
};

template <int kMode, bool kTwo>
__global__ void __launch_bounds__(kApplyThreads) bn_bwd_elemt_kernel(const __nv_bfloat16* __restrict__ g_in,
                                                                     const __nv_bfloat16* __restrict__ g2_in,
                                                                     const uint8_t* __restrict__ mask,
                                                                     const __nv_bfloat16* __restrict__ x,
                                                                     const __nv_bfloat16* __restrict__ z, ElemtArgs a,
                                                                     __nv_bfloat16* __restrict__ dx,
                                                                     __nv_bfloat16* __restrict__ dz, float norm,
                                                                     int64_t rows, int C) {
  const int groups = C / kVec;
  const int rows_per_cta = blockDim.x / groups;
  const int rsub = threadIdx.x / groups;
  if (rsub >= rows_per_cta) return;
  const int c = (threadIdx.x % groups) * kVec;
  ElemtChan p;
  elemt_params(a.mean, a.invstd, a.weight, a.sums, a.sums + C, norm, c, p);
  ElemtChan q;
  if (kMode == 2) elemt_params(a.mean_z, a.invstd_z, a.weight_z, a.sums, a.sums + 2 * C, norm, c, q);
  const int64_t step = (int64_t)gridDim.x * rows_per_cta;
#pragma unroll 2
  for (int64_t r = (int64_t)blockIdx.x * rows_per_cta + rsub; r < rows; r += step) {
    const int64_t off = r * C + c;
    uint4 vg = *reinterpret_cast<const uint4*>(g_in + off);
    if (kTwo) vg = add_bf16x8(vg, *reinterpret_cast<const uint4*>(g2_in + off));
    const unsigned mb = kMode == 1 || kMode == 3 ? 0xffu : mask[r * groups + c / kVec];
    const uint4 vx = *reinterpret_cast<const uint4*>(x + off);
    uint4 vz = make_uint4(0, 0, 0, 0);
    if (kMode == 2) vz = *reinterpret_cast<const uint4*>(z + off);
    const __nv_bfloat16* hg = reinterpret_cast<const __nv_bfloat16*>(&vg);
    const __nv_bfloat16* hx = reinterpret_cast<const __nv_bfloat16*>(&vx);
    const __nv_bfloat16* hz = reinterpret_cast<const __nv_bfloat16*>(&vz);
    uint4 vo, vd;
    __nv_bfloat16* ho = reinterpret_cast<__nv_bfloat16*>(&vo);
    __nv_bfloat16* hd = reinterpret_cast<__nv_bfloat16*>(&vd);
#pragma unroll
    for (int i = 0; i < kVec; ++i) {
      const float g = masked(hg[i], (mb >> i) & 1u);
      ho[i] = elemt(g, __bfloat162float(hx[i]), p, i, norm);
      if (kMode == 2) hd[i] = elemt(g, __bfloat162float(hz[i]), q, i, norm);
    }
    *reinterpret_cast<uint4*>(dx + off) = vo;
    if (kMode == 2) *reinterpret_cast<uint4*>(dz + off) = vd;
  }
}

__global__ void bn_update_stats_kernel(const float* __restrict__ mean, float* __restrict__ var_invstd,
                                       float* __restrict__ running_mean, float* __restrict__ running_var, int C,
                                       float momentum, float bessel, float eps) {
  const int c = blockIdx.x * blockDim.x + threadIdx.x;
  if (c >= C) return;
  const float m = mean[c], v = var_invstd[c];
  const float unbiased_var = v * bessel;
  running_mean[c] = m * momentum + (1 - momentum) * running_mean[c];
  running_var[c] = unbiased_var * momentum + (1 - momentum) * running_var[c];
  var_invstd[c] = rsqrtf(v + eps);
}

template <typename K>
cudaError_t rows_grid(K kernel, int64_t rows, int C, int& grid, int& threads) {
  const int groups = C / kVec;
  const int rows_per_cta = groups >= kApplyThreads ? 1 : kApplyThreads / groups;
  threads = groups * rows_per_cta;
  int per_sm = 0;
  cudaError_t e = cudaOccupancyMaxActiveBlocksPerMultiprocessor(&per_sm, kernel, threads, 0);
  if (e != cudaSuccess) return e;
  int64_t g = (rows + rows_per_cta - 1) / rows_per_cta;
  const int64_t cap = (int64_t)(per_sm > 0 ? per_sm : 1) * sm_count();
  grid = (int)(g > cap ? cap : g);
  return cudaSuccess;
}

template <int kMode>
cudaError_t launch_apply(const void* x, const BnParams& px, const void* z, const BnParams& pz, void* out, void* mask,
                         int64_t rows, int C, cudaStream_t st) {
  if (rows == 0) return cudaSuccess;
  int grid = 0, threads = 0;
  cudaError_t e = rows_grid(bn_apply_kernel<kMode>, rows, C, grid, threads);
  if (e != cudaSuccess) return e;
  count_launch();
  bn_apply_kernel<kMode><<<grid, threads, 0, st>>>(reinterpret_cast<const __nv_bfloat16*>(x), px,
                                                   reinterpret_cast<const __nv_bfloat16*>(z), pz,
                                                   reinterpret_cast<__nv_bfloat16*>(out),
                                                   reinterpret_cast<uint8_t*>(mask), rows, C);
  return cudaGetLastError();
}

int last_pow2(unsigned n) {
  n |= n >> 1; n |= n >> 2; n |= n >> 4; n |= n >> 8; n |= n >> 16;
  return std::max<int>(1, (int)(n - (n >> 1)));
}

RowTree row_tree(int rows, int C) {
  const int block_x = std::min(last_pow2((unsigned)C), 32);
  const int block_y = std::min(last_pow2((unsigned)((rows + 15) / 16)), 512 / block_x);
  int grid_y = std::min((rows + block_y * 16 - 1) / (block_y * 16), 128);
  if (grid_y < 8) grid_y = 1;
  return {block_y, grid_y};
}

template <int kMode, bool kTwo>
cudaError_t launch_bwd_reduce(const BnBwd& b, const RowTree& t, const BwdOut& o, int rows, int C, cudaStream_t st) {
  const int groups = C / kVec;
  const int gpc = std::min(groups, std::max(1, kReduceThreads / t.block_y));
  const dim3 grid((groups + gpc - 1) / gpc, t.grid_y);
  const int threads = gpc * t.block_y;
  count_launch();
  bn_bwd_reduce_kernel<kMode, kTwo><<<grid, threads, threads * kVec * sizeof(float), st>>>(
      reinterpret_cast<const __nv_bfloat16*>(b.go), reinterpret_cast<const __nv_bfloat16*>(b.go2), b.mask,
      reinterpret_cast<const __nv_bfloat16*>(b.x), b.px.mean, b.px.invstd, reinterpret_cast<const __nv_bfloat16*>(b.z),
      b.pz.mean, b.pz.invstd, reinterpret_cast<__nv_bfloat16*>(b.g), o, t, rows, C);
  return cudaGetLastError();
}

template <int kMode, bool kTwo>
cudaError_t launch_bwd_elemt(const BnBwd& b, const ElemtArgs& a, int64_t rows, int C, cudaStream_t st) {
  int grid = 0, threads = 0;
  cudaError_t e = rows_grid(bn_bwd_elemt_kernel<kMode, kTwo>, rows, C, grid, threads);
  if (e != cudaSuccess) return e;
  const float norm = (float)(1.0 / (double)rows);
  count_launch();
  bn_bwd_elemt_kernel<kMode, kTwo><<<grid, threads, 0, st>>>(
      reinterpret_cast<const __nv_bfloat16*>(kMode == 1 || kMode == 3 ? b.g : b.go),
      reinterpret_cast<const __nv_bfloat16*>(b.go2), b.mask, reinterpret_cast<const __nv_bfloat16*>(b.x),
      reinterpret_cast<const __nv_bfloat16*>(b.z), a, reinterpret_cast<__nv_bfloat16*>(b.dx),
      reinterpret_cast<__nv_bfloat16*>(b.dz), norm, rows, C);
  return cudaGetLastError();
}

template <int kMode, bool kTwo>
cudaError_t launch_backward(const BnBwd& b, int64_t rows64, int C, cudaStream_t st) {
  const int rows = (int)rows64;
  const RowTree t = row_tree(rows, C);
  const BwdOut o{b.sums, b.dw, b.db, b.dwz, b.dbz, b.staging};
  cudaError_t e;
  if (kMode == 3) {
    int grid = 0, threads = 0;
    e = rows_grid(bn_pool_grad_kernel<kTwo>, rows64, C, grid, threads);
    if (e != cudaSuccess) return e;
    count_launch();
    bn_pool_grad_kernel<kTwo><<<grid, threads, 0, st>>>(reinterpret_cast<const __nv_bfloat16*>(b.go),
                                                        reinterpret_cast<const __nv_bfloat16*>(b.go2), b.mask,
                                                        reinterpret_cast<__nv_bfloat16*>(b.g), b.pool, rows64, C);
    e = cudaGetLastError();
    if (e != cudaSuccess) return e;
  }
  BnBwd bb = b;
  if (kMode == 3) bb.go = b.g;
  e = launch_bwd_reduce<kMode, kTwo && kMode != 3>(bb, t, o, rows, C, st);
  if (e != cudaSuccess) return e;
  if (t.grid_y > 1) {
    const int cols = std::max(1, 512 / t.block_y);
    const int threads = cols * t.block_y;
    count_launch();
    bn_bwd_finalize_kernel<<<(C + cols - 1) / cols, threads, threads * sizeof(float), st>>>(
        o, t, kMode == 2 ? 3 : 2, C, b.px.invstd, b.pz.invstd);
    e = cudaGetLastError();
    if (e != cudaSuccess) return e;
  }
  const ElemtArgs a{b.px.mean, b.px.invstd, b.px.weight, b.sums, b.pz.mean, b.pz.invstd, b.pz.weight};
  return launch_bwd_elemt<kMode, kTwo && kMode == 2>(b, a, rows64, C, st);
}

cudaError_t launch_stats(const BnStats& s, int rows, int C, cudaStream_t st) {
  const RowTree t = row_tree(rows, C);
  const int grid_y = t.grid_y;
  const StatsOut o{s.mean, s.invstd, s.running_mean, s.running_var,
                   s.staging, s.staging + (size_t)grid_y * C, reinterpret_cast<int*>(s.staging + 2 * (size_t)grid_y * C),
                   s.momentum, s.bessel, s.eps};
  const int groups = C / kVec;
  const int gpc = std::min(groups, std::max(1, kStatsThreads / (RowTree::kLoads * t.block_y)));
  const int threads = gpc * RowTree::kLoads * t.block_y;
  count_launch();
  bn_stats_kernel<<<dim3((groups + gpc - 1) / gpc, grid_y), threads, WelfordSlots<kVec>::bytes(threads), st>>>(
      reinterpret_cast<const __nv_bfloat16*>(s.x), o, t, rows, C);
  cudaError_t e = cudaGetLastError();
  if (e != cudaSuccess || grid_y == 1) return e;
  const int cols = std::max(1, 512 / t.block_y);
  const int fthreads = cols * t.block_y;
  count_launch();
  bn_stats_finalize_kernel<<<(C + cols - 1) / cols, fthreads, WelfordSlots<1>::bytes(fthreads), st>>>(o, t, C);
  return cudaGetLastError();
}

}

void bn_row_tree(int64_t rows, int C, int* block_y, int* grid_y) {
  const RowTree t = row_tree((int)rows, C);
  *block_y = t.block_y;
  *grid_y = t.grid_y;
}

cudaError_t launch_bn_backward(int mode, const BnBwd& b, int64_t rows, int C, cudaStream_t st) {
  if (rows == 0) return cudaSuccess;
  const bool two = b.go2 != nullptr;
  switch (mode) {
    case 0: return two ? cudaErrorInvalidValue : launch_backward<0, false>(b, rows, C, st);
    case 1: return two ? launch_backward<1, true>(b, rows, C, st) : launch_backward<1, false>(b, rows, C, st);
    case 2: return two ? launch_backward<2, true>(b, rows, C, st) : launch_backward<2, false>(b, rows, C, st);
    case 3: return two ? launch_backward<3, true>(b, rows, C, st) : launch_backward<3, false>(b, rows, C, st);
    default: return cudaErrorInvalidValue;
  }
}

cudaError_t launch_bn_stats(const BnStats& s, int64_t rows, int C, cudaStream_t st) {
  if (rows == 0) return cudaSuccess;
  return launch_stats(s, (int)rows, C, st);
}

cudaError_t launch_bn_update_stats(const float* mean, float* var_invstd, float* running_mean, float* running_var, int C,
                                   float momentum, float bessel, float eps, cudaStream_t st) {
  count_launch();
  bn_update_stats_kernel<<<(C + 255) / 256, 256, 0, st>>>(mean, var_invstd, running_mean, running_var, C, momentum,
                                                          bessel, eps);
  return cudaGetLastError();
}

cudaError_t launch_bn_apply(int mode, const void* x, const BnParams& px, const void* z, const BnParams& pz, void* out,
                            void* mask, int64_t rows, int C, cudaStream_t st) {
  switch (mode) {
    case 0: return launch_apply<0>(x, px, z, pz, out, mask, rows, C, st);
    case 1: return launch_apply<1>(x, px, z, pz, out, mask, rows, C, st);
    case 2: return launch_apply<2>(x, px, z, pz, out, mask, rows, C, st);
    default: return cudaErrorInvalidValue;
  }
}

cudaError_t launch_bn_apply_pool(const void* x, const BnParams& px, void* out, void* codes, int N, const PoolGeom& pg,
                                 int C, cudaStream_t st) {
  const int64_t orows = (int64_t)N * pg.Ho * pg.Wo;
  if (orows == 0) return cudaSuccess;
  int grid = 0, threads = 0;
  cudaError_t e = rows_grid(bn_apply_pool_kernel, orows, C, grid, threads);
  if (e != cudaSuccess) return e;
  count_launch();
  bn_apply_pool_kernel<<<grid, threads, 0, st>>>(reinterpret_cast<const __nv_bfloat16*>(x), px,
                                                 reinterpret_cast<__nv_bfloat16*>(out),
                                                 reinterpret_cast<uint8_t*>(codes), orows, pg, C);
  return cudaGetLastError();
}

}
```

### deepreduce_b200/ops/csrc/ops.h

```cpp
#pragma once
#include <cuda_runtime.h>
#include <stdint.h>

#include "plan.h"

namespace dr {

int engine_max_grid(int blocks_per_sm, int dyn_smem_bytes);
cudaError_t engine_launch(const EngineParams& P, int grid, int blocks_per_sm, int dyn_smem_bytes, cudaStream_t stream);
void count_launch(int n);
long long launch_count();

struct P2Entry {
  uint32_t tensor, pos_idx, set_off, cursor, members, ord, last, tmp, misc, pair_cap;
};
struct P2Args {
  const TensorDesc* tensors;
  const TileInfo* tiles;
  const P2Entry* entries;
  uint32_t n_entries;
  uint32_t* scratch;
  uint32_t* pos_mask;
  uint32_t* tile_count;
  uint32_t* slot;
  uint32_t epoch, seed;
};
struct P2Thin {
  const TensorDesc* tensors;
  const TileInfo* tiles;
  const uint32_t* slots;
  uint32_t slot_words;
  uint32_t* dec_mask;
  int rank, world;
  uint32_t s_begin, span;
};
constexpr size_t kP2MaxSmemBytes = 128 * 1024;
cudaError_t p2_prepare();
cudaError_t p2_pick_launch(const P2Args& A, uint32_t max_pos_cap, cudaStream_t st);
cudaError_t p2_header_launch(const P2Args& A, cudaStream_t st);
cudaError_t p2_thin_launch(const P2Thin& T, cudaStream_t st);

void launch_bloom_insert(const int64_t* idx, int64_t n, uint32_t* filter, uint32_t n_hash, uint32_t m_bits,
                         uint32_t seed, cudaStream_t st);
void launch_bloom_count(const uint32_t* filter, uint32_t d, uint32_t n_hash, uint32_t m_bits, uint32_t seed,
                        uint32_t* tile_counts, uint32_t* tile_excl, cudaStream_t st);
void launch_bloom_emit(const uint32_t* filter, uint32_t d, uint32_t n_hash, uint32_t m_bits, uint32_t seed,
                       const uint32_t* tile_excl, int64_t* out, uint32_t limit, cudaStream_t st);
void launch_qsgd_encode(const float* v, int64_t K, int bucket, int q, uint32_t seed, void* lvl, bool i16, float* norms,
                        cudaStream_t st);
void launch_qsgd_decode(const void* lvl, bool i16, const float* norms, int64_t K, int bucket, int q, float* out,
                        cudaStream_t st);
void launch_pack_bits(const int64_t* vals, int64_t n, int bits, uint32_t* out, int64_t n_words, cudaStream_t st);
void launch_unpack_bits(const uint32_t* in, int64_t n_words, int64_t n, int bits, int64_t* out, cudaStream_t st);
void launch_polyfit_fit(const float* y, const int* seg_off, const int* seg_len, int n_seg, int degree, float* coeffs,
                        cudaStream_t st);
void launch_polyfit_eval(const float* coeffs, const int* seg_off, const int* seg_len, int n_seg, int degree,
                         int64_t total, float* out, cudaStream_t st);
cudaError_t launch_conflict_sets_pick(const uint32_t* set_off, const uint32_t* members, uint32_t* last, uint32_t n_sets, uint32_t n_pos,
                                      uint32_t K, uint32_t pseed, uint32_t* chosen_out, cudaStream_t st);
void launch_dexp_fit(const float* y, int64_t K, double* out_abpq, cudaStream_t st);
void launch_bp128_widths(const int64_t* idx, int64_t n, uint32_t* widths, cudaStream_t st);
void launch_bp128_pack(const int64_t* idx, int64_t n, const uint32_t* widths, const int64_t* word_off, uint32_t* out,
                       cudaStream_t st);
void launch_bp128_unpack(const uint32_t* in, int64_t n, int64_t* word_off, int64_t* deltas, cudaStream_t st);
void launch_rle_count(const int64_t* idx, int64_t n, uint32_t* counts, uint32_t* excl, cudaStream_t st);
void launch_rle_runs(const int64_t* idx, int64_t n, const uint32_t* excl, int64_t* start_pos, int64_t* end_pos,
                     int64_t n_runs, int64_t d, int64_t* runs, cudaStream_t st);
void launch_rle_expand(const int64_t* ones_excl, const int64_t* run_start, int64_t n_runs, int64_t total, int64_t* out,
                       cudaStream_t st);

cudaError_t launch_bucket_repack(bool pack, int elem_bytes, const void* src, void* dst, const int64_t* table, int n_seg,
                                 int64_t n_vec, cudaStream_t st);

struct ArenaHandle { unsigned char bytes[64]; };
void* arena_alloc(size_t bytes);
void arena_free(void* p);
ArenaHandle arena_export(void* p);
void* arena_import(const ArenaHandle& h);
void arena_close(void* p);
int arena_enable_peer_access(const int* devices, int n);
void launch_u8_to_nhwc_norm(const uint8_t* in, void* out_bf16, int64_t n_pix, const float* mean, const float* inv_std,
                            cudaStream_t st);

struct BnParams { const float* mean; const float* invstd; const float* weight; const float* bias; };
void bn_row_tree(int64_t rows, int C, int* block_y, int* grid_y);
struct BnStats {
  const void* x;
  float* mean; float* invstd; float* running_mean; float* running_var;
  float* staging;
  float momentum, bessel, eps;
};
cudaError_t launch_bn_stats(const BnStats& s, int64_t rows, int C, cudaStream_t st);
cudaError_t launch_bn_update_stats(const float* mean, float* var_invstd, float* running_mean, float* running_var, int C,
                                   float momentum, float bessel, float eps, cudaStream_t st);
cudaError_t launch_bn_apply(int mode, const void* x, const BnParams& px, const void* z, const BnParams& pz, void* out,
                            void* mask, int64_t rows, int C, cudaStream_t st);
struct PoolGeom { int H, W, Ho, Wo; };
cudaError_t launch_bn_apply_pool(const void* x, const BnParams& px, void* out, void* codes, int N, const PoolGeom& pg,
                                 int C, cudaStream_t st);
struct BnBwd {
  const void* go; const void* go2; const uint8_t* mask; const void* x; const void* z;
  BnParams px, pz;
  void* dx; void* dz; void* g;
  float* sums; float* staging; float* dw; float* db; float* dwz; float* dbz;
  PoolGeom pool;
};
cudaError_t launch_bn_backward(int mode, const BnBwd& b, int64_t rows, int C, cudaStream_t st);

}
```

### deepreduce_b200/parallel/ddp.py

```python
from __future__ import annotations

from typing import Dict, List

import torch
import torch.distributed as dist
import torch.nn as nn

from .. import spec
from ..wrappers import deepreduce_from_params
from .engine import BucketEngine
from .plan import BucketPlan


def _is_dense(p: torch.Tensor) -> bool:
    sizes, strides = list(p.size()), list(p.stride())
    expect = 1
    for st, sz in sorted(zip(strides, sizes)):
        if sz == 1:
            continue
        if st != expect:
            return False
        expect *= sz
    return True


def _fused_supported(params: dict) -> bool:
    if params.get('compressor') not in ('topk', 'threshold') or params.get('communicator', 'allgather') != 'allgather':
        return False
    dr = params.get('deepreduce', None)
    if dr is None:
        return True
    from ..codecs.bloom import canonical_policy
    policy = canonical_policy(params.get('policy', 'leftmost'))
    p2_ok = policy == 'conflict_sets' and params.get('p2_pick_mask') is True and params.get('compressor') == 'topk'
    pol_ok = policy in ('leftmost', 'random', 'p0') or p2_ok
    value_ok = (params.get('value', 'polyfit') in ('polyfit', 'bf16')
                or (params.get('value') == 'qsgd' and 1 <= int(params.get('quantum_num', 127)) <= 32767
                    and int(params.get('bucket_size', 512)) == 512))
    index = params.get('index', 'bloom')
    dexp_ok = (params.get('value') in ('dexp', 'double_exp') and params.get('fused_dexp') is True
               and ((index == 'bloom' and pol_ok) or (index == 'rle' and policy != 'conflict_sets')))
    if dr == 'index' and params.get('index', 'bloom') == 'bloom':
        return pol_ok
    if dr == 'index' and params.get('index') == 'rle':
        return True
    if dr == 'value':
        return value_ok or dexp_ok
    if dr == 'both' and params.get('index', 'bloom') == 'bloom':
        return pol_ok and (value_ok or dexp_ok)
    if dr == 'both' and params.get('index') == 'rle':
        rv, bf16 = params.get('fused_rle_values') is True, params.get('value') == 'bf16'
        return ((rv and value_ok and not bf16) or dexp_ok or (bf16 and not rv)) and policy != 'conflict_sets'
    return False


def _fused_randomk_supported(params: dict) -> bool:
    if params.get('compressor') != 'randomk' or params.get('communicator', 'allgather') not in ('allgather', 'allreduce'):
        return False
    dr = params.get('deepreduce', None)
    v = params.get('value', 'polyfit')
    return dr is None or (dr == 'value' and (v == 'bf16' or (v == 'qsgd' and 1 <= int(params.get('quantum_num', 127)) <= 32767
                                                              and int(params.get('bucket_size', 512)) == 512)))


BUCKET_DTYPES = (torch.float32, torch.bfloat16)


def group_buckets(named, cap_mb: float) -> list:
    order = list(reversed(named))
    dtypes = []
    for n, p in order:
        if p.dtype not in BUCKET_DTYPES:
            raise ValueError(f"parameter {n!r} is {p.dtype}: flat buckets hold fp32 or bf16 gradients")
        if p.dtype not in dtypes:
            dtypes.append(p.dtype)
    buckets = []
    for dt in dtypes:
        cap = int(cap_mb * 1024 * 1024 / (4 if dt == torch.float32 else 2))
        cur, cur_n = [], 0
        for n, p in order:
            if p.dtype != dt:
                continue
            if cur and cur_n + p.numel() > cap:
                buckets.append(cur)
                cur, cur_n = [], 0
            cur.append((n, p))
            cur_n += p.numel()
        if cur:
            buckets.append(cur)
    return buckets


def fused_path(params: dict) -> bool:
    return _fused_supported(params) or _fused_randomk_supported(params)


def plan_kwargs_from_params(params: dict) -> dict:
    from ..codecs.bloom import canonical_policy
    dr = params.get('deepreduce')
    v = params.get('value', 'polyfit')
    kw = dict(compress_ratio=params.get('compress_ratio', 0.01),
              index=(params.get('index', 'bloom') if dr in ('index', 'both') else None),
              value=({'double_exp': 'dexp'}.get(v, v) if dr in ('value', 'both') else None),
              quantum_num=int(params.get('quantum_num', 127)),
              poly_degree=int(params.get('poly_degree', 5)),
              fpr=params.get('fpr', None),
              policy=canonical_policy(params.get('policy', 'leftmost')),
              min_numel=int(params.get('min_numel', spec.SMALL_TENSOR_NUMEL)),
              hint=bool(params.get('hint', True)))
    if kw['value'] == 'dexp':
        from ..codecs.dexp import MIN_NUMEL
        kw['dexp_min_numel'] = int(params.get('dexp_min_numel', MIN_NUMEL))
    if params.get('compressor') == 'threshold':
        kw.update(sparsifier='threshold', threshold=float(params.get('threshold', 0.0)),
                  capacity_ratio=params.get('threshold_capacity', None))
    elif params.get('compressor') == 'randomk':
        kw.update(sparsifier='randomk')
    return kw


def engine_split_numel(params: dict, blocks_per_sm: int) -> int:
    sn = params.get('split_numel', 'auto')
    if sn == 'auto':
        uses_bloom = params.get('deepreduce') in ('index', 'both') and params.get('index', 'bloom') == 'bloom'
        from .plan import auto_split_numel
        sn = auto_split_numel(params.get('compress_ratio', 0.01), params.get('fpr', None),
                              (160 if blocks_per_sm < 2 else 80) * 1024) if uses_bloom and params.get('compressor') == 'topk' else 0
    return int(sn or 0)


def engine_kwargs(params: dict) -> dict:
    memory = params.get('memory', 'none')
    return dict(beta=float(params.get('beta', 1.0)) if memory in ('residual', 'dgc') else 0.0,
                gamma=float(params.get('gamma', 1.0)) if memory == 'residual' else 1.0,
                average=params.get('average', True),
                momentum=float(params.get('momentum', 0.9)) if memory == 'dgc' else None,
                weight_decay=float(params.get('weight_decay', 0.0)) if memory == 'dgc' else 0.0)


def make_engine(plan: BucketPlan, params: dict, *, device, group, use_history: bool, blocks_per_sm: int,
                grad_dtype: torch.dtype, parameters=None, owner=None) -> BucketEngine:
    eng = BucketEngine(plan, device=device, group=group, use_history=use_history, blocks_per_sm=blocks_per_sm,
                       grad_dtype=grad_dtype, **engine_kwargs(params))
    if eng.weight_decay != 0.0:
        if parameters is None:
            raise ValueError("'weight_decay' reads the parameters: make_engine needs the bucket's parameters")
        eng.bind_parameters(parameters, owner)
    if params.get('calibrate_partition', True) and eng.cuts is not None:
        try:
            eng.calibrate_partition()
        except (ValueError, ArithmeticError, IndexError) as e:
            import warnings
            warnings.warn(f"deepreduce_b200: partition calibration skipped ({e!r}); using the static cut")
            eng.cta_speeds = None
            eng._set_cuts()
            eng.resid.zero_(); eng.sel.zero_(); eng.grad.zero_()
            if eng.mom is not None:
                eng.mom.zero_()
    return eng


class DeepReduceDDP:
    def __init__(self, module: nn.Module, params: dict, *, bucket_cap_mb: float = 1e9, overlap: bool = True,
                 group=None, blocks_per_sm: int = 2, use_history: bool = True, background_thread: bool = True,
                 broadcast_parameters: bool = True, overlap_grid: int | None = None):
        self.module = module
        self.params = dict(params)
        self.group = group
        self.world = dist.get_world_size(group) if dist.is_initialized() else 1
        self.rank = dist.get_rank(group) if dist.is_initialized() else 0
        self.named = [(n, p) for n, p in module.named_parameters() if p.requires_grad]
        self.device = self.named[0][1].device
        self.is_cuda = self.device.type == "cuda"
        self.dense = self.params.get('compressor', 'none') in ('none', None)
        self.fused = self.is_cuda and not self.dense and fused_path(self.params)
        self.overlap = overlap and self.is_cuda
        self.step_count = 0
        self.engines: List[BucketEngine] = []
        self.flat: List[torch.Tensor] = []
        self.bucket_of: Dict[int, int] = {}
        self.pending: List[int] = []
        self.sched = None
        self.grc = None
        self._handles = []
        self._exchange = True
        self._grad_views: Dict[int, torch.Tensor] = {}
        self._status_host = None
        self._status_event = None
        self.overlap_grid_cap = int(overlap_grid if overlap_grid is not None else (self.params.get('overlap_grid', 0) or 0))
        if self.world > 1 and broadcast_parameters:
            with torch.no_grad():
                for t in list(module.parameters()) + list(module.buffers()):
                    dist.broadcast(t.data, 0, group=group)
        if self.fused or (self.dense and self.is_cuda):
            self._build_buckets(bucket_cap_mb, blocks_per_sm, use_history)
            if (self.fused and self.overlap and background_thread
                    and all(e.transport == "p2p" for e in self.engines)):
                from .. import ops
                self.sched = ops.cuda_module().Scheduler(len(self.buckets))
            if self.overlap:
                self._install_hooks()
        else:
            self.grc = deepreduce_from_params(self.params)
            if hasattr(self.grc.memory, "bind_parameters"):
                self.grc.memory.bind_parameters(self.named)

    def _build_buckets(self, cap_mb, blocks_per_sm, use_history):
        self.buckets: List[List] = group_buckets(self.named, cap_mb)
        for b, items in enumerate(self.buckets):
            dtype = items[0][1].dtype
            numels = [p.numel() for _, p in items]
            names = [n for n, _ in items]
            shapes = [tuple(p.shape) for _, p in items]
            owner = list(range(len(items)))
            if self.fused:
                sn = engine_split_numel(self.params, blocks_per_sm)
                if sn:
                    from .plan import split_large
                    numels, names, shapes, owner = split_large(numels, names, shapes, int(sn))
            if self.fused:
                plan = BucketPlan(numels, names, shapes, **plan_kwargs_from_params(self.params))
                eng = make_engine(plan, self.params, device=self.device, group=self.group, use_history=use_history,
                                  blocks_per_sm=blocks_per_sm, grad_dtype=dtype, parameters=[p for _, p in items],
                                  owner=owner)
                self.engines.append(eng)
                flat, views = eng.grad, eng.grad_views
            else:
                plan = BucketPlan(numels, names, shapes, index=None)
                flat = torch.zeros(plan.total_elems, dtype=dtype, device=self.device)
                views = plan.views(flat)
            self.flat.append(flat)
            first = {}
            for j, o in enumerate(owner):
                first.setdefault(o, plan.tensors[j])
            for i, (n, p) in enumerate(items):
                t = first[i]
                seg = flat[t.elem_off:t.elem_off + p.numel()]
                p.grad = seg.as_strided(p.size(), p.stride()) if _is_dense(p) else seg.view(p.shape)
                self._grad_views[id(p)] = p.grad
                self.bucket_of[id(p)] = b
        self._in_backward = False
        self._ready_count = [0] * len(self.buckets)
        self._launched = [False] * len(self.buckets)
        self._bucket_size = [len(it) for it in self.buckets]

    def _install_hooks(self):
        for n, p in self.named:
            self._handles.append(p.register_post_accumulate_grad_hook(self._hook))

    def set_exchange_enabled(self, on: bool):
        self._exchange = bool(on)

    def _hook(self, p):
        if not self._exchange:
            return
        b = self.bucket_of[id(p)]
        self._ready_count[b] += 1
        if self._ready_count[b] == self._bucket_size[b]:
            self._in_backward = True
            try:
                self._launch_bucket(b)
            finally:
                self._in_backward = False

    def _launch_bucket(self, b):
        self._ready_count[b] = 0
        self._launched[b] = True
        if self.fused:
            eng = self.engines[b]
            eng.refresh_parameters()
            eng.epoch = eng.epoch + 1
            more_to_come = not all(self._launched)
            if self.sched is not None and more_to_come:
                eng.ctx.set_grid_cap(self.overlap_grid_cap if self.overlap_grid_cap > 0 else 0)
                self.sched.submit(b, eng.ctx, eng.epoch)
            else:
                eng.ctx.set_grid_cap(0)
                if self.sched is not None and len(self.buckets) > 1 and self.world > 1:
                    self.sched.wait_all()
                eng.step(eng.epoch)
        else:
            if self.world > 1:
                self.pending.append(dist.all_reduce(self.flat[b], group=self.group, async_op=True))

    def zero_grad(self):
        if self.flat:
            for f in self.flat:
                f.zero_()
        else:
            for _, p in self.named:
                p.grad = None

    def finish(self):
        if self.grc is not None:
            for n, p in self.named:
                if p.grad is not None:
                    p.grad = self.grc.step(p.grad, n).view_as(p)
        elif self.fused:
            self._check_grad_views()
            for b in range(len(self.buckets)):
                if not self._launched[b]:
                    self._launch_bucket(b)
            if self.sched is not None:
                self.sched.wait_all()
            self._launched = [False] * len(self.buckets)
        else:
            self._check_grad_views()
            for b in range(len(self.buckets)):
                if not self._launched[b]:
                    self._launch_bucket(b)
            self._launched = [False] * len(self.buckets)
            for w in self.pending:
                w.wait()
            self.pending = []
            if self.world > 1 and self.params.get('average', True):
                for f in self.flat:
                    f.div_(self.world)
        self.step_count += 1

    def _check_grad_views(self):
        for _, p in self.named:
            v = self._grad_views.get(id(p))
            if v is None or p.grad is v:
                continue
            if p.grad is None:
                v.zero_()
            elif p.grad.data_ptr() != v.data_ptr():
                v.copy_(p.grad)
            p.grad = v

    def check_async(self):
        if not self.engines:
            return
        if self._status_host is not None and self._status_event.query():
            st = self._status_host
            for b in range(len(self.engines)):
                if int(st[b, 0]) != 0:
                    from .engine import STATUS_NAMES
                    raise RuntimeError(f"[rank {self.rank}/{self.world}] bucket {b} (step {self.step_count}): deepreduce "
                                       f"engine error: {STATUS_NAMES.get(int(st[b, 0]), int(st[b, 0]))} (aux={int(st[b, 1])})")
        if self._status_host is None:
            self._status_host = torch.zeros(len(self.engines), 8, dtype=torch.int32).pin_memory()
            self._status_event = torch.cuda.Event()
        for b, e in enumerate(self.engines):
            self._status_host[b].copy_(e.status, non_blocking=True)
        self._status_event.record()

    def check(self):
        for b, e in enumerate(self.engines):
            try:
                e.check_status()
            except RuntimeError as err:
                raise RuntimeError(f"[rank {self.rank}/{self.world}] bucket {b} "
                                   f"({len(self.buckets[b])} tensors, step {self.step_count}): {err}") from err

    def wire_bytes_per_step(self) -> int:
        if self.fused:
            return sum(e.plan.wire_bytes() for e in self.engines)
        if self.dense:
            return sum(f.numel() * f.element_size() for f in self.flat)
        return int(self.grc.bytes_sent / max(self.step_count, 1))

    def stage2_bytes_per_step(self) -> int:
        if not self.fused or self.world == 1:
            return 0
        torch.cuda.synchronize(self.device)
        return sum(e.stage2_bytes() for e in self.engines)

    def dense_bytes(self) -> int:
        return sum(p.numel() * p.element_size() for _, p in self.named)

    def exchange_stats(self) -> dict:
        if not self.fused:
            return {"wire_bytes": self.wire_bytes_per_step(), "dense_bytes": self.dense_bytes()}
        torch.cuda.synchronize(self.device)
        tot: dict = {}
        for e in self.engines:
            for k, v in e.stats()["total"].items():
                tot[k] = tot.get(k, 0) + v
        tot["relative_volume"] = tot["wire_bytes"] / max(1, tot["dense_bytes"])
        return tot

    def state_dict(self):
        if self.fused:
            return {"step": self.step_count, "engines": [e.state_dict() for e in self.engines]}
        if self.grc is not None:
            return {"step": self.step_count, "memory": self.grc.memory.state_dict()}
        return {"step": self.step_count}

    def load_state_dict(self, state):
        self.step_count = int(state.get("step", 0))
        if self.fused:
            for e, s in zip(self.engines, state["engines"]):
                e.load_state_dict(s)
        elif self.grc is not None and "memory" in state:
            self.grc.memory.load_state_dict(state["memory"], device=self.device)

    def close(self):
        for h in self._handles:
            h.remove()
        if self.sched is not None:
            self.sched.shutdown()
            self.sched = None
        for e in self.engines:
            e.close()
```

### deepreduce_b200/trainer.py

```python
from __future__ import annotations

from typing import Callable, Optional

import torch
import torch.nn as nn
import torch.nn.functional as F

from .parallel.ddp import DeepReduceDDP


class Trainer:
    def __init__(self, model: nn.Module, params: dict, *, lr: float = 0.1, momentum: float = 0.9,
                 weight_decay: float = 1e-4, amp_dtype: Optional[torch.dtype] = torch.bfloat16,
                 channels_last: bool = False, loss_fn: Optional[Callable] = None, optimizer=None,
                 overlap: bool = True, bucket_cap_mb: float = 1e9, background_thread: bool = True,
                 blocks_per_sm: int = 2, u8_input: bool = False, accum_steps: int = 1, nvtx: bool = False,
                 check_every: int = 100, overlap_grid: Optional[int] = None):
        self.model = model
        self.device = next(model.parameters()).device
        self.is_cuda = self.device.type == "cuda"
        self.amp_dtype = amp_dtype if self.is_cuda else None
        self.channels_last = channels_last and self.is_cuda
        if self.channels_last:
            self.model = self.model.to(memory_format=torch.channels_last)
        self.loss_fn = loss_fn or F.cross_entropy
        self.ddp = DeepReduceDDP(self.model, params, overlap=overlap, bucket_cap_mb=bucket_cap_mb,
                                 background_thread=background_thread, blocks_per_sm=blocks_per_sm,
                                 overlap_grid=overlap_grid)
        if optimizer is None:
            if params.get('memory') == 'dgc':
                momentum = 0.0
                if 'weight_decay' in params:
                    weight_decay = 0.0
            kw = dict(lr=lr, momentum=momentum, weight_decay=weight_decay)
            if self.is_cuda:
                kw["fused"] = True
            optimizer = torch.optim.SGD(self.model.parameters(), **kw)
        self.opt = optimizer
        self.u8_input = u8_input
        self.accum_steps = max(1, int(accum_steps))
        self._micro = 0
        self.check_every = max(0, int(check_every))
        self._opt_steps = 0
        self.nvtx = nvtx and self.is_cuda
        self._copy_stream = torch.cuda.Stream(device=self.device) if self.is_cuda else None
        self._staged = None
        self._loss_host = torch.zeros(1, dtype=torch.float32).pin_memory() if self.is_cuda else torch.zeros(1)
        self.h2d_bytes = 0
        self.d2h_bytes = 0

    def _prep(self, x):
        if self.u8_input and x.dtype == torch.uint8:
            from . import ops
            x = ops.u8_to_nhwc_norm(x).permute(0, 3, 1, 2)
        elif self.channels_last and x.dim() == 4:
            x = x.contiguous(memory_format=torch.channels_last)
        return x

    def _range(self, name):
        import contextlib
        return torch.cuda.nvtx.range(name) if self.nvtx else contextlib.nullcontext()

    def step(self, *inputs, target) -> torch.Tensor:
        first = self._micro == 0
        last = self._micro == self.accum_steps - 1
        if first:
            self.ddp.zero_grad()
        self.ddp.set_exchange_enabled(last)
        inputs = tuple(self._prep(x) for x in inputs)
        with self._range("forward"):
            if self.amp_dtype is not None:
                with torch.autocast(device_type="cuda", dtype=self.amp_dtype):
                    out = self.model(*inputs)
            else:
                out = self.model(*inputs)
            loss = self.loss_fn(out.float() if torch.is_tensor(out) and out.is_floating_point() else out, target)
        with self._range("backward+exchange"):
            (loss / self.accum_steps if self.accum_steps > 1 else loss).backward()
        self._micro = (self._micro + 1) % self.accum_steps
        if last:
            with self._range("finish+optimizer"):
                self.ddp.finish()
                self.opt.step()
            self._opt_steps += 1
            if self.is_cuda:
                self.ddp.check_async()
            if self.check_every and self._opt_steps % self.check_every == 0:
                self.ddp.check()
        return loss.detach()

    def _stage(self, host_inputs, host_target):
        with torch.cuda.stream(self._copy_stream):
            dev = tuple(t.to(self.device, non_blocking=True) for t in host_inputs)
            tgt = host_target.to(self.device, non_blocking=True)
            ev = torch.cuda.Event()
            ev.record(self._copy_stream)
        self.h2d_bytes = sum(t.numel() * t.element_size() for t in host_inputs) + host_target.numel() * host_target.element_size()
        return dev, tgt, ev

    def step_host(self, host_inputs, host_target, next_batch=None) -> float:
        if not self.is_cuda:
            return float(self.step(*host_inputs, target=host_target))
        if self._staged is None:
            self._staged = self._stage(host_inputs, host_target)
        dev, tgt, ev = self._staged
        torch.cuda.current_stream().wait_event(ev)
        self._staged = self._stage(*next_batch) if next_batch is not None else None
        loss = self.step(*dev, target=tgt)
        self._loss_host.copy_(loss.reshape(1), non_blocking=True)
        self.d2h_bytes = 4
        torch.cuda.current_stream().synchronize()
        for t in dev:
            t.record_stream(torch.cuda.current_stream())
        return float(self._loss_host[0])

    def close(self):
        self.ddp.close()
```

Before: 6173.

## Cast conv/linear weights to bf16 in one batched kernel and land grads in buckets

Adds a WeightShadow that casts all fp32 conv and linear weights to a flat bf16 buffer with one batched kernel per step, replacing autocast's per-layer weight casts. Backward gradients for shadowed weights and BN affine params are written or accumulated directly into the DDP bucket views, and the DDP layer is signalled through a landing callback instead of relying on AccumulateGrad hooks. The BN num_batches_tracked increment is folded into the stats kernel. The aim is fewer small cast, copy and accumulate kernels per step, at the cost of extra bf16 weight memory and more complex hook bookkeeping that could break gradient-ready ordering.

```diff
diff --git a/deepreduce_b200/models/fused_bn.py b/deepreduce_b200/models/fused_bn.py
--- a/deepreduce_b200/models/fused_bn.py
+++ b/deepreduce_b200/models/fused_bn.py
@@ -26,10 +26,101 @@
     return enabled() and _eligible_x(x) and _eligible_bn(bn)
 
 
+_LANDING = {}
+
+
+def register_landing(p: torch.Tensor, view: torch.Tensor, landed) -> None:
+    _LANDING[id(p)] = (p, view, landed)
+
+
+def unregister_landing(p: torch.Tensor) -> None:
+    _LANDING.pop(id(p), None)
+
+
+def landing(p: torch.Tensor):
+    e = _LANDING.get(id(p))
+    if e is None or e[0] is not p or p.grad is not e[1]:
+        return None
+    return e[1], e[2]
+
+
+def landings(params):
+    out = []
+    for p in params:
+        e = landing(p)
+        if e is None:
+            return None
+        out.append((p, *e))
+    return out
+
+
+def _land(land, grads):
+    if land is None:
+        return grads
+    for p, _, landed in land:
+        landed(p)
+    return (None,) * len(grads)
+
+
+def _views(land):
+    return [] if land is None else [v for _, v, _ in land]
+
+
+class WeightShadow:
+
+    def __init__(self, params):
+        self.params = list(params)
+        offs, n = [], 0
+        for p in self.params:
+            offs.append(n)
+            n += -(-p.numel() // 8) * 8
+        self.flat = torch.empty(n, dtype=torch.bfloat16, device=self.params[0].device)
+        self._views = {id(p): self.flat[o:o + p.numel()].as_strided(p.size(), p.stride())
+                       for p, o in zip(self.params, offs)}
+        self._key = None
+        self._native = None
+
+    def refresh(self) -> None:
+        from .. import ops
+        key = [(p.data_ptr(), p.stride()) for p in self.params]
+        if key != self._key:
+            for p in self.params:
+                if p.stride() != self._views[id(p)].stride():
+                    v = self._views[id(p)]
+                    self._views[id(p)] = v.as_strided(p.size(), p.stride(), v.storage_offset())
+            self._native = ops.cuda_module().Bf16Shadow(self.params, [self._views[id(p)] for p in self.params])
+            self._key = key
+        self._native.run()
+
+    def active(self):
+        import contextlib
+
+        @contextlib.contextmanager
+        def ctx():
+            self.refresh()
+            global _SHADOW
+            prev, _SHADOW = _SHADOW, self
+            try:
+                yield self
+            finally:
+                _SHADOW = prev
+        return ctx()
+
+    def view(self, p: torch.Tensor):
+        return self._views.get(id(p))
+
+
+_SHADOW = None
+
+
+def shadow_view(p: torch.Tensor):
+    return None if _SHADOW is None else _SHADOW.view(p)
+
+
 def _stats(x, bn):
     from .. import ops
-    bn.num_batches_tracked.add_(1)
-    return ops.cuda_module().bn_stats(x, bn.running_mean, bn.running_var, float(bn.momentum), float(bn.eps))
+    return ops.cuda_module().bn_stats(x, bn.running_mean, bn.running_var, float(bn.momentum), float(bn.eps),
+                                      num_batches_tracked=bn.num_batches_tracked)
 
 
 def _grad(go):
@@ -50,26 +141,28 @@
 
 class _BNReLU(torch.autograd.Function):
     @staticmethod
-    def forward(ctx, x, weight, bias, mean, invstd):
+    def forward(ctx, x, weight, bias, mean, invstd, land):
         from .. import ops
         y, mask = ops.cuda_module().bn_apply(0, x, [mean, invstd, weight, bias])
         ctx.save_for_backward(x, weight, mean, invstd, mask)
+        ctx.land = land
         return y
 
     @staticmethod
     def backward(ctx, gy):
         from .. import ops
         x, weight, mean, invstd, mask = ctx.saved_tensors
-        dx, dw, db = ops.cuda_module().bn_backward(0, _grad(gy), mask, x, [mean, invstd, weight])
-        return dx, dw, db, None, None
+        dx, dw, db = ops.cuda_module().bn_backward(0, _grad(gy), mask, x, [mean, invstd, weight], grads=_views(ctx.land))
+        return (dx, *_land(ctx.land, (dw, db)), None, None, None)
 
 
 class _BNAddReLU(torch.autograd.Function):
 
     @staticmethod
-    def forward(ctx, x, weight, bias, mean, invstd, z, wz, bz, mz, iz, fork):
+    def forward(ctx, x, weight, bias, mean, invstd, z, wz, bz, mz, iz, fork, land):
         from .. import ops
         mod = ops.cuda_module()
+        ctx.land = land
         if wz is None:
             o, mask = mod.bn_apply(1, x, [mean, invstd, weight, bias], z)
             ctx.save_for_backward(x, weight, mean, invstd, mask)
@@ -85,24 +178,28 @@
         mod = ops.cuda_module()
         go, go2 = _grads(grads)
         if go is None:
-            return (None,) * 11
+            return (None,) * 12
         saved = ctx.saved_tensors
         x, weight, mean, invstd, mask = saved[:5]
         if not ctx.has_bn_z:
-            dx, dw, db, g = mod.bn_backward(1, go, mask, x, [mean, invstd, weight], go2=go2)
-            return dx, dw, db, None, None, g, None, None, None, None, None
+            dx, dw, db, g = mod.bn_backward(1, go, mask, x, [mean, invstd, weight], go2=go2, grads=_views(ctx.land))
+            dw, db = _land(ctx.land, (dw, db))
+            return dx, dw, db, None, None, g, None, None, None, None, None, None
         z, wz, mz, iz = saved[5:]
-        dx, dw, db, dz, dwz, dbz = mod.bn_backward(2, go, mask, x, [mean, invstd, weight], z, [mz, iz, wz], go2=go2)
-        return dx, dw, db, None, None, dz, dwz, dbz, None, None, None
+        dx, dw, db, dz, dwz, dbz = mod.bn_backward(2, go, mask, x, [mean, invstd, weight], z, [mz, iz, wz], go2=go2,
+                                                   grads=_views(ctx.land))
+        dw, db, dwz, dbz = _land(ctx.land, (dw, db, dwz, dbz))
+        return dx, dw, db, None, None, dz, dwz, dbz, None, None, None, None
 
 
 class _BNReLUMaxPool(torch.autograd.Function):
 
     @staticmethod
-    def forward(ctx, x, weight, bias, mean, invstd, fork):
+    def forward(ctx, x, weight, bias, mean, invstd, fork, land):
         from .. import ops
         out, codes = ops.cuda_module().bn_apply_pool(x, [mean, invstd, weight, bias])
         ctx.save_for_backward(x, weight, mean, invstd, codes)
+        ctx.land = land
         return _fork(ctx, out, fork)
 
     @staticmethod
@@ -110,10 +207,11 @@
         from .. import ops
         go, go2 = _grads(grads)
         if go is None:
-            return (None,) * 6
+            return (None,) * 7
         x, weight, mean, invstd, codes = ctx.saved_tensors
-        dx, dw, db = ops.cuda_module().bn_backward(3, go, codes, x, [mean, invstd, weight], go2=go2)
-        return dx, dw, db, None, None, None
+        dx, dw, db = ops.cuda_module().bn_backward(3, go, codes, x, [mean, invstd, weight], go2=go2,
+                                                   grads=_views(ctx.land))
+        return (dx, *_land(ctx.land, (dw, db)), None, None, None, None)
 
 
 def _stem_pool(pool: nn.Module) -> bool:
@@ -132,21 +230,22 @@
     if not (eligible(x, bn) and _stem_pool(pool)):
         return _pair(pool(F.relu(bn(x), inplace=True)), fork)
     mean, invstd = _stats(x, bn)
-    return _BNReLUMaxPool.apply(x, bn.weight, bn.bias, mean, invstd, fork)
+    return _BNReLUMaxPool.apply(x, bn.weight, bn.bias, mean, invstd, fork, landings((bn.weight, bn.bias)))
 
 
 def bn_relu(x: torch.Tensor, bn: nn.BatchNorm2d) -> torch.Tensor:
     if not eligible(x, bn):
         return F.relu(bn(x), inplace=True)
     mean, invstd = _stats(x, bn)
-    return _BNReLU.apply(x, bn.weight, bn.bias, mean, invstd)
+    return _BNReLU.apply(x, bn.weight, bn.bias, mean, invstd, landings((bn.weight, bn.bias)))
 
 
 def bn_add_relu(x: torch.Tensor, bn: nn.BatchNorm2d, idt: torch.Tensor, fork: bool = False):
     if not (eligible(x, bn) and idt.dtype == x.dtype and idt.shape == x.shape and idt.stride() == x.stride()):
         return _pair(F.relu(bn(x) + idt, inplace=True), fork)
     mean, invstd = _stats(x, bn)
-    return _BNAddReLU.apply(x, bn.weight, bn.bias, mean, invstd, idt, None, None, None, None, fork)
+    return _BNAddReLU.apply(x, bn.weight, bn.bias, mean, invstd, idt, None, None, None, None, fork,
+                            landings((bn.weight, bn.bias)))
 
 
 def bn_bn_add_relu(x: torch.Tensor, bn: nn.BatchNorm2d, xd: torch.Tensor, bnd: nn.BatchNorm2d, fork: bool = False):
@@ -154,4 +253,5 @@
         return _pair(F.relu(bn(x) + bnd(xd), inplace=True), fork)
     md, id_ = _stats(xd, bnd)
     mean, invstd = _stats(x, bn)
-    return _BNAddReLU.apply(x, bn.weight, bn.bias, mean, invstd, xd, bnd.weight, bnd.bias, md, id_, fork)
+    return _BNAddReLU.apply(x, bn.weight, bn.bias, mean, invstd, xd, bnd.weight, bnd.bias, md, id_, fork,
+                            landings((bn.weight, bn.bias, bnd.weight, bnd.bias)))
diff --git a/deepreduce_b200/models/resnet.py b/deepreduce_b200/models/resnet.py
--- a/deepreduce_b200/models/resnet.py
+++ b/deepreduce_b200/models/resnet.py
@@ -1,9 +1,55 @@
 from __future__ import annotations
 
+import torch
 import torch.nn as nn
 import torch.nn.functional as F
 
+from . import fused_bn
 from .fused_bn import bn_add_relu, bn_bn_add_relu, bn_relu, bn_relu_maxpool
+
+
+class _Shadow(torch.autograd.Function):
+    @staticmethod
+    def forward(ctx, p, w16, land):
+        ctx.land = land
+        return w16.detach()
+
+    @staticmethod
+    def backward(ctx, g):
+        from .. import ops
+        p, view, landed = ctx.land
+        if g.stride() != view.stride():
+            g = torch.empty_strided(view.size(), view.stride(), dtype=g.dtype, device=g.device).copy_(g)
+        ops.cuda_module().grad_land(view, g)
+        landed(p)
+        return None, None, None
+
+
+def _shadowed(p):
+    w16 = fused_bn.shadow_view(p)
+    land = None if w16 is None else fused_bn.landing(p)
+    return None if land is None else _Shadow.apply(p, w16, (p, *land))
+
+
+def _training_bf16(m: nn.Module) -> bool:
+    return (m.training and fused_bn.enabled() and torch.is_autocast_enabled("cuda")
+            and torch.get_autocast_dtype("cuda") == torch.bfloat16)
+
+
+def conv(x, m: nn.Conv2d):
+    if type(m) is nn.Conv2d and m.bias is None and _training_bf16(m):
+        w16 = _shadowed(m.weight)
+        if w16 is not None:
+            return m._conv_forward(x, w16, None)
+    return m(x)
+
+
+def linear(x, m: nn.Linear):
+    if type(m) is nn.Linear and m.bias is not None and _training_bf16(m):
+        w16, b16 = _shadowed(m.weight), _shadowed(m.bias)
+        if w16 is not None and b16 is not None:
+            return F.linear(x, w16, b16)
+    return m(x)
 
 
 class _BasicCifar(nn.Module):
@@ -68,10 +114,10 @@
 
     def forward(self, x, skip=None, fork=False):
         skip = x if skip is None else skip
-        xd = None if self.downsample is None else self.downsample[0](skip)
-        y = bn_relu(self.conv1(x), self.bn1)
-        y = bn_relu(self.conv2(y), self.bn2)
-        y = self.conv3(y)
+        xd = None if self.downsample is None else conv(skip, self.downsample[0])
+        y = bn_relu(conv(x, self.conv1), self.bn1)
+        y = bn_relu(conv(y, self.conv2), self.bn2)
+        y = conv(y, self.conv3)
         if xd is None:
             return bn_add_relu(y, self.bn3, skip, fork=fork)
         o = bn_bn_add_relu(y, self.bn3, xd, self.downsample[1])
@@ -97,11 +143,11 @@
                 nn.init.kaiming_normal_(m.weight, mode="fan_out", nonlinearity="relu")
 
     def forward(self, x):
-        x, skip = bn_relu_maxpool(self.conv1(x), self.bn1, self.maxpool), None
+        x, skip = bn_relu_maxpool(conv(x, self.conv1), self.bn1, self.maxpool), None
         for blk in self.layers:
             x, skip = blk(x, skip, fork=True)
         x = F.adaptive_avg_pool2d(x, 1).flatten(1)
-        return self.fc(x)
+        return linear(x, self.fc)
 
 
 def resnet50(num_classes: int = 1000) -> ResNet:
diff --git a/deepreduce_b200/ops/build.py b/deepreduce_b200/ops/build.py
--- a/deepreduce_b200/ops/build.py
+++ b/deepreduce_b200/ops/build.py
@@ -11,7 +11,7 @@
 CSRC = os.path.join(HERE, "csrc")
 OBJ = os.path.join(HERE, "build")
 
-CUDA_SOURCES = ["engine.cu", "ops.cu", "p2p.cu", "bn.cu", "p2.cu", "repack.cu"]
+CUDA_SOURCES = ["engine.cu", "ops.cu", "p2p.cu", "bn.cu", "p2.cu", "repack.cu", "params.cu"]
 NVCC_FLAGS = ["-gencode", "arch=compute_90a,code=sm_90a", "-lineinfo", "-O3", "-std=c++17",
               "--expt-relaxed-constexpr", "--expt-extended-lambda", "-Xcompiler", "-fPIC", "-Xptxas", "-v"]
 
diff --git a/deepreduce_b200/ops/csrc/binding.cpp b/deepreduce_b200/ops/csrc/binding.cpp
--- a/deepreduce_b200/ops/csrc/binding.cpp
+++ b/deepreduce_b200/ops/csrc/binding.cpp
@@ -328,11 +328,19 @@
 }
 
 static std::vector<torch::Tensor> bn_stats(torch::Tensor x, torch::Tensor running_mean, torch::Tensor running_var,
-                                           double momentum, double eps, bool torch_kernel) {
+                                           double momentum, double eps, bool torch_kernel,
+                                           c10::optional<torch::Tensor> num_batches_tracked) {
   check_bn_input(x);
   const int64_t C = x.size(1);
   check_chan(running_mean, C, "running_mean");
   check_chan(running_var, C, "running_var");
+  int64_t* counter = nullptr;
+  if (num_batches_tracked.has_value()) {
+    const torch::Tensor& t = *num_batches_tracked;
+    TORCH_CHECK(t.device() == x.device() && t.scalar_type() == torch::kInt64 && t.numel() == 1,
+                "bn_stats: num_batches_tracked must be an int64 scalar on x's device");
+    counter = t.data_ptr<int64_t>();
+  }
   const int64_t N = x.numel() / C;
   TORCH_CHECK(N > 1, "bn: expected more than 1 value per channel when training");
   c10::cuda::CUDAGuard g(x.device());
@@ -346,12 +354,12 @@
     auto staging = grid_y > 1 ? torch::empty({(2 * C + 1) * grid_y}, opts) : torch::Tensor();
     const dr::BnStats s{x.data_ptr(), mean.data_ptr<float>(), invstd.data_ptr<float>(), running_mean.data_ptr<float>(),
                         running_var.data_ptr<float>(), grid_y > 1 ? staging.data_ptr<float>() : nullptr,
-                        (float)momentum, bessel, (float)eps};
+                        (float)momentum, bessel, (float)eps, counter};
     e = dr::launch_bn_stats(s, N, (int)C, cur_stream());
   } else {
     at::native::batch_norm_stats_channels_last_cuda_template<c10::BFloat16, at::native::Var>(mean, invstd, x, eps);
     e = dr::launch_bn_update_stats(mean.data_ptr<float>(), invstd.data_ptr<float>(), running_mean.data_ptr<float>(),
-                                   running_var.data_ptr<float>(), (int)C, (float)momentum, bessel, (float)eps,
+                                   running_var.data_ptr<float>(), (int)C, (float)momentum, bessel, (float)eps, counter,
                                    cur_stream());
   }
   TORCH_CHECK(e == cudaSuccess, "bn_stats: ", cudaGetErrorString(e));
@@ -420,7 +428,8 @@
 
 static std::vector<torch::Tensor> bn_backward(int64_t mode, torch::Tensor go, torch::Tensor mask, torch::Tensor x,
                                               std::vector<torch::Tensor> p, c10::optional<torch::Tensor> z,
-                                              std::vector<torch::Tensor> pz, c10::optional<torch::Tensor> go2) {
+                                              std::vector<torch::Tensor> pz, c10::optional<torch::Tensor> go2,
+                                              std::vector<torch::Tensor> grads) {
   TORCH_CHECK(mode >= 0 && mode <= 3, "bn_backward: mode must be 0, 1, 2 or 3");
   TORCH_CHECK(!go2.has_value() || mode != 0, "bn_backward: mode 0 takes no go2");
   check_bn_input(x);
@@ -445,8 +454,17 @@
   auto f32 = x.options().dtype(torch::kFloat32);
   auto sums = torch::empty({n_sums, C}, f32);
   auto staging = grid_y > 1 ? torch::empty({n_sums, grid_y, C}, f32) : torch::Tensor();
-  auto dx = torch::empty_like(x), dw = torch::empty({C}, f32), db = torch::empty({C}, f32);
+  const size_t n_grads = mode == 2 ? 4 : 2;
+  TORCH_CHECK(grads.empty() || grads.size() == n_grads, "bn_backward: grads must be (dw, db) or, for mode 2, (dw, db, "
+              "dw_z, db_z)");
+  for (const auto& t : grads) check_chan(t, C, "each of grads");
+  for (size_t i = 0; i < grads.size(); ++i)
+    for (size_t j = 0; j < i; ++j)
+      TORCH_CHECK(grads[i].data_ptr() != grads[j].data_ptr(), "bn_backward: grads must be distinct buffers");
+  const bool acc = !grads.empty();
+  auto dx = torch::empty_like(x), dw = acc ? grads[0] : torch::empty({C}, f32), db = acc ? grads[1] : torch::empty({C}, f32);
   dr::BnBwd b{};
+  b.accumulate = acc;
   b.go = go.data_ptr(); b.go2 = go2.has_value() ? go2->data_ptr() : nullptr; b.mask = mask.data_ptr<uint8_t>(); b.x = x.data_ptr();
   b.px = bn_bwd_params(p, C);
   b.dx = dx.data_ptr(); b.sums = sums.data_ptr<float>(); b.staging = grid_y > 1 ? staging.data_ptr<float>() : nullptr;
@@ -463,13 +481,62 @@
     check_like_x(*z, x, "z");
     b.z = z->data_ptr();
     b.pz = bn_bwd_params(pz, C);
-    auto dz = torch::empty_like(x), dwz = torch::empty({C}, f32), dbz = torch::empty({C}, f32);
+    auto dz = torch::empty_like(x), dwz = acc ? grads[2] : torch::empty({C}, f32), dbz = acc ? grads[3] : torch::empty({C}, f32);
     b.dz = dz.data_ptr(); b.dwz = dwz.data_ptr<float>(); b.dbz = dbz.data_ptr<float>();
     res.insert(res.end(), {dz, dwz, dbz});
   }
   cudaError_t e = dr::launch_bn_backward((int)mode, b, rows, (int)C, cur_stream());
   TORCH_CHECK(e == cudaSuccess, "bn_backward: ", cudaGetErrorString(e));
   return res;
+}
+
+struct Bf16Shadow {
+  std::vector<torch::Tensor> src, dst;
+  torch::Tensor table;
+  int64_t n_blocks = 0;
+
+  Bf16Shadow(std::vector<torch::Tensor> s, std::vector<torch::Tensor> d) : src(std::move(s)), dst(std::move(d)) {
+    TORCH_CHECK(!src.empty() && src.size() == dst.size(), "Bf16Shadow: expected as many destinations as sources");
+    std::vector<int64_t> rows;
+    std::vector<std::pair<uintptr_t, uintptr_t>> spans;
+    for (size_t i = 0; i < src.size(); ++i) {
+      const auto &a = src[i], &b = dst[i];
+      TORCH_CHECK(a.is_cuda() && a.scalar_type() == torch::kFloat32 && b.scalar_type() == torch::kBFloat16 &&
+                      b.device() == a.device() && a.device() == src[0].device(),
+                  "Bf16Shadow: fp32 sources and bf16 destinations on one CUDA device");
+      TORCH_CHECK(a.sizes() == b.sizes() && a.strides() == b.strides() && a.is_non_overlapping_and_dense() &&
+                      b.is_non_overlapping_and_dense(),
+                  "Bf16Shadow: each destination must have its source's sizes and strides, both dense");
+      const int64_t n = a.numel();
+      rows.insert(rows.end(), {(int64_t)reinterpret_cast<uintptr_t>(a.data_ptr()),
+                               (int64_t)reinterpret_cast<uintptr_t>(b.data_ptr()), n, n_blocks});
+      n_blocks += (n + dr::kShadowChunk - 1) / dr::kShadowChunk;
+      const uintptr_t p = reinterpret_cast<uintptr_t>(b.data_ptr());
+      spans.push_back({p, p + 2 * (uintptr_t)n});
+    }
+    std::sort(spans.begin(), spans.end());
+    for (size_t i = 1; i < spans.size(); ++i)
+      TORCH_CHECK(spans[i].first >= spans[i - 1].second, "Bf16Shadow: destinations overlap");
+    TORCH_CHECK(n_blocks < (int64_t{1} << 31), "Bf16Shadow: too many elements");
+    table = torch::tensor(rows, torch::dtype(torch::kInt64)).view({-1, 4}).to(src[0].device());
+  }
+
+  void run() {
+    c10::cuda::CUDAGuard g(table.device());
+    cudaError_t e = dr::launch_bf16_shadow(table.data_ptr<int64_t>(), (int)src.size(), n_blocks, cur_stream());
+    TORCH_CHECK(e == cudaSuccess, "Bf16Shadow: ", cudaGetErrorString(e));
+  }
+};
+
+static void grad_land(torch::Tensor dst, torch::Tensor g) {
+  TORCH_CHECK(dst.is_cuda() && dst.scalar_type() == torch::kFloat32 && g.scalar_type() == torch::kBFloat16 &&
+                  g.device() == dst.device(),
+              "grad_land: expected an fp32 destination and a bf16 gradient on one CUDA device");
+  TORCH_CHECK(dst.sizes() == g.sizes() && dst.strides() == g.strides() && dst.is_non_overlapping_and_dense(),
+              "grad_land: the gradient must have the destination's sizes and strides, both dense");
+  c10::cuda::CUDAGuard guard(dst.device());
+  cudaError_t e = dr::launch_grad_land(dst.data_ptr<float>(), g.data_ptr(), dst.numel(), cur_stream());
+  TORCH_CHECK(e == cudaSuccess, "grad_land: ", cudaGetErrorString(e));
 }
 
 struct Engine {
@@ -754,13 +821,17 @@
   m.def("delta_bp128_decode", &delta_bp128_decode);
   m.def("u8_to_nhwc_norm", &u8_to_nhwc_norm);
   m.def("bn_stats", &bn_stats, py::arg("x"), py::arg("running_mean"), py::arg("running_var"), py::arg("momentum"),
-        py::arg("eps"), py::arg("torch_kernel") = false);
+        py::arg("eps"), py::arg("torch_kernel") = false, py::arg("num_batches_tracked") = py::none());
   m.def("bn_apply", &bn_apply, py::arg("mode"), py::arg("x"), py::arg("p"), py::arg("z") = py::none(),
         py::arg("pz") = std::vector<torch::Tensor>{});
   m.def("bn_apply_pool", &bn_apply_pool, py::arg("x"), py::arg("p"), py::arg("kernel_size") = 3, py::arg("stride") = 2,
         py::arg("padding") = 1, py::arg("dilation") = 1, py::arg("ceil_mode") = false);
   m.def("bn_backward", &bn_backward, py::arg("mode"), py::arg("go"), py::arg("mask"), py::arg("x"), py::arg("p"),
-        py::arg("z") = py::none(), py::arg("pz") = std::vector<torch::Tensor>{}, py::arg("go2") = py::none());
+        py::arg("z") = py::none(), py::arg("pz") = std::vector<torch::Tensor>{}, py::arg("go2") = py::none(),
+        py::arg("grads") = std::vector<torch::Tensor>{});
+  py::class_<Bf16Shadow>(m, "Bf16Shadow").def(py::init<std::vector<torch::Tensor>, std::vector<torch::Tensor>>())
+      .def("run", &Bf16Shadow::run);
+  m.def("grad_land", &grad_land);
   m.def("rle_runs", &rle_runs);
   m.def("rle_indices", &rle_indices);
   m.def("arena_alloc", &arena_alloc);
diff --git a/deepreduce_b200/ops/csrc/bn.cu b/deepreduce_b200/ops/csrc/bn.cu
--- a/deepreduce_b200/ops/csrc/bn.cu
+++ b/deepreduce_b200/ops/csrc/bn.cu
@@ -312,6 +312,7 @@
   float* mean; float* invstd; float* running_mean; float* running_var;
   float* st_mean; float* st_m2n; int* st_count;
   float momentum, bessel, eps;
+  int64_t* counter;
 };
 
 __device__ __forceinline__ void stats_store(const StatsOut& o, int c, int n, float mean, float m2n) {
@@ -321,6 +322,7 @@
   o.invstd[c] = rsqrtf(__fadd_rn(var, o.eps));
   o.running_mean[c] = __fmaf_rn(mean, o.momentum, __fmul_rn(o.running_mean[c], keep));
   o.running_var[c] = __fmaf_rn(__fmul_rn(var, o.bessel), o.momentum, __fmul_rn(o.running_var[c], keep));
+  if (c == 0 && o.counter) *o.counter += 1;
 }
 
 __global__ void __launch_bounds__(kStatsThreads) bn_stats_kernel(const __nv_bfloat16* __restrict__ x, StatsOut o,
@@ -427,18 +429,23 @@
   float* sums;
   float* dw; float* db; float* dwz; float* dbz;
   float* staging;
+  bool accumulate;
 };
+
+__device__ __forceinline__ void param_store(const BwdOut& o, float* p, int c, float v) {
+  p[c] = o.accumulate ? __fadd_rn(p[c], v) : v;
+}
 
 __device__ __forceinline__ void bwd_store(const BwdOut& o, int k, int c, int C, float v, const float* invstd,
                                          const float* invstd_z) {
   o.sums[k * C + c] = v;
   if (k == 0) {
-    o.db[c] = v;
-    if (o.dbz) o.dbz[c] = v;
+    param_store(o, o.db, c, v);
+    if (o.dbz) param_store(o, o.dbz, c, v);
   } else if (k == 1) {
-    o.dw[c] = __fmul_rn(v, invstd[c]);
+    param_store(o, o.dw, c, __fmul_rn(v, invstd[c]));
   } else {
-    o.dwz[c] = __fmul_rn(v, invstd_z[c]);
+    param_store(o, o.dwz, c, __fmul_rn(v, invstd_z[c]));
   }
 }
 
@@ -643,9 +650,10 @@
 
 __global__ void bn_update_stats_kernel(const float* __restrict__ mean, float* __restrict__ var_invstd,
                                        float* __restrict__ running_mean, float* __restrict__ running_var, int C,
-                                       float momentum, float bessel, float eps) {
+                                       float momentum, float bessel, float eps, int64_t* __restrict__ counter) {
   const int c = blockIdx.x * blockDim.x + threadIdx.x;
   if (c >= C) return;
+  if (c == 0 && counter) *counter += 1;
   const float m = mean[c], v = var_invstd[c];
   const float unbiased_var = v * bessel;
   running_mean[c] = m * momentum + (1 - momentum) * running_mean[c];
@@ -728,7 +736,7 @@
 cudaError_t launch_backward(const BnBwd& b, int64_t rows64, int C, cudaStream_t st) {
   const int rows = (int)rows64;
   const RowTree t = row_tree(rows, C);
-  const BwdOut o{b.sums, b.dw, b.db, b.dwz, b.dbz, b.staging};
+  const BwdOut o{b.sums, b.dw, b.db, b.dwz, b.dbz, b.staging, b.accumulate};
   cudaError_t e;
   if (kMode == 3) {
     int grid = 0, threads = 0;
@@ -763,7 +771,7 @@
   const int grid_y = t.grid_y;
   const StatsOut o{s.mean, s.invstd, s.running_mean, s.running_var,
                    s.staging, s.staging + (size_t)grid_y * C, reinterpret_cast<int*>(s.staging + 2 * (size_t)grid_y * C),
-                   s.momentum, s.bessel, s.eps};
+                   s.momentum, s.bessel, s.eps, s.counter};
   const int groups = C / kVec;
   const int gpc = std::min(groups, std::max(1, kStatsThreads / (RowTree::kLoads * t.block_y)));
   const int threads = gpc * RowTree::kLoads * t.block_y;
@@ -805,10 +813,10 @@
 }
 
 cudaError_t launch_bn_update_stats(const float* mean, float* var_invstd, float* running_mean, float* running_var, int C,
-                                   float momentum, float bessel, float eps, cudaStream_t st) {
+                                   float momentum, float bessel, float eps, int64_t* counter, cudaStream_t st) {
   count_launch();
   bn_update_stats_kernel<<<(C + 255) / 256, 256, 0, st>>>(mean, var_invstd, running_mean, running_var, C, momentum,
-                                                          bessel, eps);
+                                                          bessel, eps, counter);
   return cudaGetLastError();
 }
 
diff --git a/deepreduce_b200/ops/csrc/ops.h b/deepreduce_b200/ops/csrc/ops.h
--- a/deepreduce_b200/ops/csrc/ops.h
+++ b/deepreduce_b200/ops/csrc/ops.h
@@ -89,10 +89,11 @@
   float* mean; float* invstd; float* running_mean; float* running_var;
   float* staging;
   float momentum, bessel, eps;
+  int64_t* counter;
 };
 cudaError_t launch_bn_stats(const BnStats& s, int64_t rows, int C, cudaStream_t st);
 cudaError_t launch_bn_update_stats(const float* mean, float* var_invstd, float* running_mean, float* running_var, int C,
-                                   float momentum, float bessel, float eps, cudaStream_t st);
+                                   float momentum, float bessel, float eps, int64_t* counter, cudaStream_t st);
 cudaError_t launch_bn_apply(int mode, const void* x, const BnParams& px, const void* z, const BnParams& pz, void* out,
                             void* mask, int64_t rows, int C, cudaStream_t st);
 struct PoolGeom { int H, W, Ho, Wo; };
@@ -104,7 +105,12 @@
   void* dx; void* dz; void* g;
   float* sums; float* staging; float* dw; float* db; float* dwz; float* dbz;
   PoolGeom pool;
+  bool accumulate;
 };
 cudaError_t launch_bn_backward(int mode, const BnBwd& b, int64_t rows, int C, cudaStream_t st);
 
+constexpr int64_t kShadowChunk = 8192;
+cudaError_t launch_bf16_shadow(const int64_t* table, int n_rows, int64_t n_blocks, cudaStream_t st);
+cudaError_t launch_grad_land(float* dst, const void* g, int64_t n, cudaStream_t st);
+
 }
diff --git a/deepreduce_b200/ops/csrc/params.cu b/deepreduce_b200/ops/csrc/params.cu
--- /dev/null
+++ b/deepreduce_b200/ops/csrc/params.cu
@@ -0,0 +1,92 @@
+#include <cuda_bf16.h>
+#include <cuda_runtime.h>
+
+#include <cstdint>
+
+#include "common.cuh"
+#include "ops.h"
+
+namespace dr {
+
+namespace {
+
+constexpr int kCastThreads = 256;
+constexpr int kLandThreads = 256;
+
+__device__ __forceinline__ int shadow_row(const int64_t* __restrict__ tab, int n_rows, int64_t b) {
+  int lo = 0, hi = n_rows - 1;
+  while (lo < hi) {
+    const int mid = (lo + hi + 1) >> 1;
+    if (__ldg(tab + 4 * mid + 3) <= b) lo = mid; else hi = mid - 1;
+  }
+  return lo;
+}
+
+__global__ void __launch_bounds__(kCastThreads) bf16_shadow_kernel(const int64_t* __restrict__ tab, int n_rows) {
+  const int r = shadow_row(tab, n_rows, blockIdx.x);
+  const float* src = reinterpret_cast<const float*>(__ldg(tab + 4 * r));
+  __nv_bfloat16* dst = reinterpret_cast<__nv_bfloat16*>(__ldg(tab + 4 * r + 1));
+  const int64_t n = __ldg(tab + 4 * r + 2);
+  const int64_t begin = (blockIdx.x - __ldg(tab + 4 * r + 3)) * kShadowChunk;
+  const int64_t end = begin + kShadowChunk < n ? begin + kShadowChunk : n;
+  int64_t tail = begin;
+  if (((reinterpret_cast<uintptr_t>(src) & 15) | (reinterpret_cast<uintptr_t>(dst) & 7)) == 0) {
+    const int64_t vend = begin + ((end - begin) & ~int64_t(3));
+    for (int64_t i = begin + 4 * threadIdx.x; i < vend; i += 4 * kCastThreads) {
+      const float4 v = *reinterpret_cast<const float4*>(src + i);
+      const __nv_bfloat162 lo = __halves2bfloat162(__float2bfloat16(v.x), __float2bfloat16(v.y));
+      const __nv_bfloat162 hi = __halves2bfloat162(__float2bfloat16(v.z), __float2bfloat16(v.w));
+      *reinterpret_cast<uint2*>(dst + i) =
+          make_uint2(*reinterpret_cast<const uint32_t*>(&lo), *reinterpret_cast<const uint32_t*>(&hi));
+    }
+    tail = vend;
+  }
+  for (int64_t i = tail + threadIdx.x; i < end; i += kCastThreads) dst[i] = __float2bfloat16(src[i]);
+}
+
+__global__ void __launch_bounds__(kLandThreads) grad_land_kernel(float* __restrict__ dst,
+                                                                 const __nv_bfloat16* __restrict__ g, int64_t n,
+                                                                 bool vec) {
+  const int64_t stride = (int64_t)gridDim.x * kLandThreads;
+  int64_t tail = 0;
+  if (vec) {
+    const int64_t nv = n / 8;
+    for (int64_t v = (int64_t)blockIdx.x * kLandThreads + threadIdx.x; v < nv; v += stride) {
+      const uint4 gv = *reinterpret_cast<const uint4*>(g + 8 * v);
+      const __nv_bfloat16* hg = reinterpret_cast<const __nv_bfloat16*>(&gv);
+      float4* d = reinterpret_cast<float4*>(dst + 8 * v);
+      float4 a = d[0], b = d[1];
+      a.x = __fadd_rn(a.x, __bfloat162float(hg[0])); a.y = __fadd_rn(a.y, __bfloat162float(hg[1]));
+      a.z = __fadd_rn(a.z, __bfloat162float(hg[2])); a.w = __fadd_rn(a.w, __bfloat162float(hg[3]));
+      b.x = __fadd_rn(b.x, __bfloat162float(hg[4])); b.y = __fadd_rn(b.y, __bfloat162float(hg[5]));
+      b.z = __fadd_rn(b.z, __bfloat162float(hg[6])); b.w = __fadd_rn(b.w, __bfloat162float(hg[7]));
+      d[0] = a;
+      d[1] = b;
+    }
+    tail = nv * 8;
+  }
+  for (int64_t i = tail + (int64_t)blockIdx.x * kLandThreads + threadIdx.x; i < n; i += stride)
+    dst[i] = __fadd_rn(dst[i], __bfloat162float(g[i]));
+}
+
+}
+
+cudaError_t launch_bf16_shadow(const int64_t* table, int n_rows, int64_t n_blocks, cudaStream_t st) {
+  if (n_rows == 0 || n_blocks == 0) return cudaSuccess;
+  count_launch();
+  bf16_shadow_kernel<<<(unsigned)n_blocks, kCastThreads, 0, st>>>(table, n_rows);
+  return cudaGetLastError();
+}
+
+cudaError_t launch_grad_land(float* dst, const void* g, int64_t n, cudaStream_t st) {
+  if (n == 0) return cudaSuccess;
+  const bool vec = ((reinterpret_cast<uintptr_t>(dst) | reinterpret_cast<uintptr_t>(g)) & 15) == 0;
+  const int64_t work = vec ? (n + 7) / 8 : n;
+  const int64_t grid = (work + kLandThreads - 1) / kLandThreads;
+  count_launch();
+  grad_land_kernel<<<(unsigned)(grid < 4096 ? grid : 4096), kLandThreads, 0, st>>>(
+      dst, reinterpret_cast<const __nv_bfloat16*>(g), n, vec);
+  return cudaGetLastError();
+}
+
+}
diff --git a/deepreduce_b200/parallel/ddp.py b/deepreduce_b200/parallel/ddp.py
--- a/deepreduce_b200/parallel/ddp.py
+++ b/deepreduce_b200/parallel/ddp.py
@@ -7,6 +7,7 @@
 import torch.nn as nn
 
 from .. import spec
+from ..models import fused_bn
 from ..wrappers import deepreduce_from_params
 from .engine import BucketEngine
 from .plan import BucketPlan
@@ -185,6 +186,7 @@
         self._handles = []
         self._exchange = True
         self._grad_views: Dict[int, torch.Tensor] = {}
+        self._landed = set()
         self._status_host = None
         self._status_event = None
         self.overlap_grid_cap = int(overlap_grid if overlap_grid is not None else (self.params.get('overlap_grid', 0) or 0))
@@ -239,6 +241,7 @@
                 p.grad = seg.as_strided(p.size(), p.stride()) if _is_dense(p) else seg.view(p.shape)
                 self._grad_views[id(p)] = p.grad
                 self.bucket_of[id(p)] = b
+                fused_bn.register_landing(p, p.grad, self.landed)
         self._in_backward = False
         self._ready_count = [0] * len(self.buckets)
         self._launched = [False] * len(self.buckets)
@@ -252,6 +255,11 @@
         self._exchange = bool(on)
 
     def _hook(self, p):
+        if id(p) in self._landed:
+            return
+        self._ready(p)
+
+    def _ready(self, p):
         if not self._exchange:
             return
         b = self.bucket_of[id(p)]
@@ -262,6 +270,11 @@
                 self._launch_bucket(b)
             finally:
                 self._in_backward = False
+
+    def landed(self, p):
+        self._landed.add(id(p))
+        if self._handles:
+            self._ready(p)
 
     def _launch_bucket(self, b):
         self._ready_count[b] = 0
@@ -292,6 +305,7 @@
                 p.grad = None
 
     def finish(self):
+        self._landed.clear()
         if self.grc is not None:
             for n, p in self.named:
                 if p.grad is not None:
@@ -397,6 +411,8 @@
             self.grc.memory.load_state_dict(state["memory"], device=self.device)
 
     def close(self):
+        for _, p in self.named:
+            fused_bn.unregister_landing(p)
         for h in self._handles:
             h.remove()
         if self.sched is not None:
diff --git a/deepreduce_b200/trainer.py b/deepreduce_b200/trainer.py
--- a/deepreduce_b200/trainer.py
+++ b/deepreduce_b200/trainer.py
@@ -1,11 +1,13 @@
 from __future__ import annotations
 
+import contextlib
 from typing import Callable, Optional
 
 import torch
 import torch.nn as nn
 import torch.nn.functional as F
 
+from .models import fused_bn
 from .parallel.ddp import DeepReduceDDP
 
 
@@ -37,6 +39,12 @@
                 kw["fused"] = True
             optimizer = torch.optim.SGD(self.model.parameters(), **kw)
         self.opt = optimizer
+        self.shadow = None
+        if self.amp_dtype == torch.bfloat16 and fused_bn.enabled():
+            ps = [p for m in self.model.modules() if isinstance(m, (nn.Conv2d, nn.Linear))
+                  for p in m.parameters(recurse=False)
+                  if p.dtype == torch.float32 and fused_bn.landing(p) is not None]
+            self.shadow = fused_bn.WeightShadow(ps) if ps else None
         self.u8_input = u8_input
         self.accum_steps = max(1, int(accum_steps))
         self._micro = 0
@@ -58,7 +66,6 @@
         return x
 
     def _range(self, name):
-        import contextlib
         return torch.cuda.nvtx.range(name) if self.nvtx else contextlib.nullcontext()
 
     def step(self, *inputs, target) -> torch.Tensor:
@@ -70,7 +77,8 @@
         inputs = tuple(self._prep(x) for x in inputs)
         with self._range("forward"):
             if self.amp_dtype is not None:
-                with torch.autocast(device_type="cuda", dtype=self.amp_dtype):
+                shadow = self.shadow.active() if self.shadow is not None else contextlib.nullcontext()
+                with torch.autocast(device_type="cuda", dtype=self.amp_dtype), shadow:
                     out = self.model(*inputs)
             else:
                 out = self.model(*inputs)
```

New measurement: 6298, median of 6. 1.02x the previous value.
